# mantasu/face-crop-plus

Hardware: AMD Instinct MI355X
Metric: faces/sec end-to-end (detect+align+crop) (higher is better)
Workload: dtype f16x3; 1 GPU; RetinaFace detect + 5-pt align/crop, batch=32/GPU synthetic 1024x1024 RGB, strategy=largest, det_threshold=0.6, output 256x256, detector on 2 HIP streams x 16 images; global_batch=32, image_size=1024, parallelism=dp1

## Files before the change

face-crop-plus_amd/_native.py:

```python
from __future__ import annotations

import ctypes as C
import os

_HERE = os.path.dirname(os.path.abspath(__file__))
LIB_PATH = os.path.join(_HERE, "csrc", "libfcp_hip.so")
ABI_VERSION = 15

c_f32p = C.c_void_p
_lib = None


class ConvDesc(C.Structure):
    _fields_ = [
        ("in_", C.c_void_p), ("w", C.c_void_p), ("bias", C.c_void_p), ("out", C.c_void_p),
        ("res1", C.c_void_p), ("res2", C.c_void_p), ("wscale", C.c_void_p), ("in2", C.c_void_p),
        ("n", C.c_int32), ("in_h", C.c_int32), ("in_w", C.c_int32),
        ("cin", C.c_int32), ("in_ld", C.c_int32), ("in_up2", C.c_int32),
        ("cout", C.c_int32), ("kh", C.c_int32), ("kw", C.c_int32),
        ("stride", C.c_int32), ("pad", C.c_int32),
        ("out_h", C.c_int32), ("out_w", C.c_int32), ("out_ld", C.c_int32),
        ("tile_n", C.c_int32), ("cin4", C.c_int32),
        ("act_slope", C.c_float), ("alpha", C.c_float), ("alpha2", C.c_float),
        ("res1_pre", C.c_int32), ("res1_ld", C.c_int32), ("res1_h", C.c_int32),
        ("res1_w", C.c_int32), ("res2_ld", C.c_int32), ("precision", C.c_int32),
        ("in_fmt", C.c_int32), ("out_fmt", C.c_int32), ("res1_fmt", C.c_int32), ("res2_fmt", C.c_int32),
        ("tile_m", C.c_int32), ("cin2", C.c_int32), ("in2_ld", C.c_int32), ("in2_h", C.c_int32),
        ("in2_w", C.c_int32), ("in2_stride", C.c_int32), ("flags", C.c_int32), ("cu_budget", C.c_int32),
        ("band_top", C.c_int32), ("band_bottom", C.c_int32),
    ]


CONV_FLAT_ADDR = 1
CONV_BALANCE_TAIL = 2
CHAIN_OUT_EVEN_ONLY = 1


class ChainDesc(C.Structure):
    _fields_ = [(k, C.c_void_p) for k in ("t1", "w2", "ws2", "b2", "w3", "ws3", "b3", "res", "out", "w1n", "ws1n",
                                          "b1n", "t1n", "t1b")] + \
               [(k, C.c_int32) for k in ("n", "h", "w", "c", "cn", "t1_ld", "res_ld", "out_ld", "t1n_ld", "nout", "tile_m", "flags",
                                         "cb", "t1b_ld", "t1b_h", "t1b_w", "t1b_stride")]


_P, _I, _F, _L = C.c_void_p, C.c_int, C.c_float, C.c_int64
SIGNATURES = {
    "fcp_conv2d_nhwc_f32": [C.POINTER(ConvDesc), _P],
    "fcp_bottleneck_chain_f16x3": [C.POINTER(ChainDesc), _P],
    "fcp_u8_to_nhwc4_f32": [_P, _P, _L, C.POINTER(C.c_float), _F, _P],
    "fcp_f32nchw_to_nhwc4_f32": [_P, _P, _I, _I, _I, C.POINTER(C.c_float), _F, _P],
    "fcp_maxpool3x3s2_nhwc_f32": [_P, _P, _I, _I, _I, _I, _I, _I, _I, _P],
    "fcp_maxpool3x3s2_split32": [_P, _P, _I, _I, _I, _I, _I, _I, _I, _P],
    "fcp_stem7x7s2_relu_pool_u8": [_P, _I, _I, _I, C.POINTER(C.c_int32), _P, _P, _P, _P, _I, _I, _P],
    "fcp_stem7x7s2_relu_pool_conv1_u8": [_P, _I, _I, _I, C.POINTER(C.c_int32), _P, _P, _P, _P, _I, _I, _P, _P, _P, _P, _I, _P],
    "fcp_stem7x7s2_relu_pool_f32": [_P, _I, _I, _I, _P, _P, _P, _P, _I, _I, _P],
    "fcp_f32_to_split32": [_P, _P, _L, _I, _P],
    "fcp_split32_to_f32": [_P, _P, _L, _I, _P],
    "fcp_absmax_nhwc": [_P, _L, _I, _I, _I, _P, _P],
    "fcp_retina_decode": [_P, _P, _P, _I, _I, _I, _F, _F, _F, _P, _P, _P, _P, _P, _P, _P, _P, _P],
    "fcp_retina_nms_select": [_P, _P, _P, _I, _I, _F, _I, _P, _P, _P, _P, _P, _P],
    "fcp_retina_gather_faces": [_P, _P, _P, _I, _I, _P, _I, _P, _P, _P, _P],
    "fcp_estimate_transform": [_P, _P, _I, _I, _I, _P, _P, _P],
    "fcp_estimate_transform_counted": [_P, _P, _I, _I, _I, _P, _P, _P, _P, _P],
    "fcp_bise_preprocess_u8": [_P, _I, _I, _I, _P, _I, _I, C.POINTER(C.c_float), C.POINTER(C.c_float), _P],
    "fcp_avgpool_nhwc_f32": [_P, _I, _I, _I, _I, _P, _P],
    "fcp_fc_f32": [_P, _P, _P, _P, _I, _I, _I, _I, _P, _P],
    "fcp_scale_add_nhwc_f32": [_P, _I, _P, _P, _P, _I, _I, _I, _I, _P, _I, _P],
    "fcp_parse_tail": [_P, _I, _I, _I, _I, _I, _I, _I, _I, _I, _P, _P, _P],
    "fcp_label_mask_u8": [_P, _L, C.c_uint32, _P, _P],
    "fcp_bicubic_down4_u8": [_P, _I, _I, _I, _P, _P],
    "fcp_warp_affine_u8": [_P, _I, _I, _I, _P, _P, _P, _P, _I, _I, _I, _I, _P, _P],
    "fcp_warp_affine_u8_float": [_P, _I, _I, _I, _P, _P, _P, _P, _I, _I, _I, _I, _P, _P],
    "fcp_build_batch_u8": [_P, _L, _P, _P, _I, _I, _I, _I, _P, _P],
    "fcp_warp_affine_u8_ragged": [_P, _L, _P, _P, _P, _P, _I, _I, _I, _I, _P, _P],
    "fcp_warp_affine_u8_float_ragged": [_P, _L, _P, _P, _P, _P, _I, _I, _I, _I, _P, _P],
    "fcp_resize_area_ragged_u8": [_P, _L, _P, _P, _I, _P, _L, _P],
    "fcp_warp_affine_u8_interp": [_P, _I, _I, _I, _P, _P, _P, _P, _I, _I, _I, _I, _I, _P, _P],
    "fcp_warp_affine_u8_interp_ragged": [_P, _L, _P, _P, _P, _P, _I, _I, _I, _I, _I, _P, _P],
    "fcp_warp_interp_weights": [_I, _P],
    "fcp_crop_sharpness_u8": [_P, _I, _I, _I, _P, _P, _P],
    "fcp_jpeg_encode_u8": [_P, _I, _I, _I, _I, _I, _I, _P, _L, _L, _P, _P, _L, _P],
    "fcp_jpeg_encode_ex_u8": [_P, _I, _I, _I, _I, _I, _I, _I, _P, _L, _L, _P, _P, _P, _L, _P],
    "fcp_jpeg_huffman_tables": [_P, _I, _P, _P, _P],
    "fcp_png_encode_u8": [_P, _I, _I, _I, _I, _P, _L, _L, _P, _P, _L, _P],
    "fcp_png_huffman_lengths": [_P, _I, _P, _P, _P],
    "fcp_matte_u8": [_P, _P, _I, _I, _I, C.c_uint32, _I, _I, _I, _I, _P, _P, _P],
    "fcp_clahe_u8": [_P, _I, _I, _I, _I, C.c_double, _P, _P, _P],
    "fcp_matte_blur_u8": [_P, _P, _I, _I, _I, C.c_uint32, _I, _P, _I, _P, _P, _P, _L, _P],
    "fcp_matte_refine_u8": [_P, _P, _I, _I, _I, C.c_uint32, _I, _I, _P, _P, _L, _P],
    "fcp_matte_alpha_u8": [_P, _P, _I, _I, _I, _I, _I, _I, _P, _P],
    "fcp_matte_blur_alpha_u8": [_P, _P, _P, _I, _I, _I, C.c_uint32, _P, _I, _P, _P, _L, _P],
    "fcp_subject_mask_u8": [_P, _I, _I, _I, C.c_uint32, _I, _I, _P, _P, _L, _P],
    "fcp_feather_alpha_u8": [_P, _I, _I, _I, C.c_uint32, _I, _P, _P],
    "fcp_cutout_u8": [_P, _P, _I, _I, _I, _I, _I, _I, _I, _P, _I, _P, _P, _L, _P],
}
EXPORTS = ["fcp_abi_version", "fcp_last_error", "fcp_retina_nms_workspace_bytes", "fcp_jpeg_workspace_bytes",
           "fcp_jpeg_workspace_bytes_ex", "fcp_matte_blur_workspace_bytes", "fcp_matte_refine_workspace_bytes",
           "fcp_subject_mask_workspace_bytes", "fcp_png_workspace_bytes", "fcp_cutout_workspace_bytes"] + list(SIGNATURES)


def lib():
    global _lib
    if _lib is not None:
        return _lib
    if not os.path.isfile(LIB_PATH):
        raise RuntimeError(
            f"HIP extension not built: {LIB_PATH} is missing. Run "
            f"`python face-crop-plus_amd/build_native.py` (needs hipcc). There is no CPU fallback.")
    l = C.CDLL(LIB_PATH)
    l.fcp_abi_version.restype = C.c_int
    l.fcp_last_error.restype = C.c_char_p
    if l.fcp_abi_version() != ABI_VERSION:
        raise RuntimeError(f"libfcp_hip.so ABI {l.fcp_abi_version()} != expected {ABI_VERSION}; rebuild")
    l.fcp_retina_nms_workspace_bytes.argtypes = [C.c_int, C.c_int]
    l.fcp_retina_nms_workspace_bytes.restype = C.c_int64
    l.fcp_jpeg_workspace_bytes.argtypes = [C.c_int, C.c_int, C.c_int, C.c_int]
    l.fcp_jpeg_workspace_bytes.restype = C.c_int64
    l.fcp_jpeg_workspace_bytes_ex.argtypes = [C.c_int] * 6
    l.fcp_jpeg_workspace_bytes_ex.restype = C.c_int64
    l.fcp_png_workspace_bytes.argtypes = [C.c_int, C.c_int, C.c_int, C.c_int]
    l.fcp_png_workspace_bytes.restype = C.c_int64
    l.fcp_matte_blur_workspace_bytes.argtypes = [C.c_int, C.c_int, C.c_int]
    l.fcp_matte_blur_workspace_bytes.restype = C.c_int64
    l.fcp_matte_refine_workspace_bytes.argtypes = [C.c_int, C.c_int, C.c_int]
    l.fcp_matte_refine_workspace_bytes.restype = C.c_int64
    l.fcp_subject_mask_workspace_bytes.argtypes = [C.c_int, C.c_int, C.c_int]
    l.fcp_subject_mask_workspace_bytes.restype = C.c_int64
    l.fcp_cutout_workspace_bytes.argtypes = [C.c_int, C.c_int, C.c_int]
    l.fcp_cutout_workspace_bytes.restype = C.c_int64
    for name, args in SIGNATURES.items():
        fn = getattr(l, name)
        fn.argtypes = args
        fn.restype = C.c_int
    _lib = l
    return l


def check(rc: int, what: str = ""):
    if rc != 0:
        msg = lib().fcp_last_error().decode(errors="replace")
        raise RuntimeError(f"{what or 'fcp_hip'} failed ({rc}): {msg}")


def stream_ptr():
    import torch
    return C.c_void_p(torch.cuda.current_stream().cuda_stream)


def ptr(t, byte_offset: int = 0):
    if t is None:
        return C.c_void_p(0)
    return C.c_void_p(t.data_ptr() + byte_offset)
```

face-crop-plus_amd/csrc/fcp_retina_post.hip:

```cpp
#include "fcp_common.h"
#include "fcp_hip.h"

namespace {

constexpr int DEC_THREADS = 1024;
constexpr int NMS_THREADS = 1024;
constexpr int SORT_LDS_KEYS = 8192;
constexpr int NMS_ALIVE_WORDS = SORT_LDS_KEYS - 256;
constexpr int NMS_LDS_CAP = NMS_ALIVE_WORDS * 64;
constexpr int NMS_MAX_CAP = 1 << 26;

struct Levels {
  int h[3], w[3], start[4];
};

__device__ __forceinline__ int ceil_div(int a, int b) { return (a + b - 1) / b; }

constexpr int DEC_MAX_ROUNDS = 64;

struct Decoded {
  float score, box[4], ldm[10];
};

__device__ __forceinline__ const float* head_cell(const float* head0, const float* head1, const float* head2, const Levels& lv,
                                                  int img, int p, int& l, int& cell, int& a) {
  l = p >= lv.start[2] ? 2 : (p >= lv.start[1] ? 1 : 0);
  const int q = p - lv.start[l];
  cell = q >> 1; a = q & 1;
  return (l == 0 ? head0 : (l == 1 ? head1 : head2)) + ((long)img * lv.h[l] * lv.w[l] + cell) * 32;
}

__device__ __forceinline__ float face_score(const float* hp, int a) {
  const float l0 = hp[2 * a], l1 = hp[2 * a + 1];
  const float mx = fmaxf(l0, l1);
  const float e0 = expf(l0 - mx), e1 = expf(l1 - mx);
  const float inv = 1.0f / (e0 + e1);
  return e1 * inv;
}

__device__ __forceinline__ void decode_prior(const float* hp, const Levels& lv, int l, int cell, int a, int img_h, int img_w,
                                             float v0, float v1, Decoded& d) {
  const float fw = (float)img_w, fh = (float)img_h;
  const int wl = lv.w[l];
  const int i = cell / wl, j = cell - i * wl;
  const int step = 8 << l;
  const double ms = (double)((16 << (2 * l)) << a);
  const float pcx = (float)(((double)j + 0.5) * (double)step / (double)img_w);
  const float pcy = (float)(((double)i + 0.5) * (double)step / (double)img_h);
  const float pw = (float)(ms / (double)img_w);
  const float ph = (float)(ms / (double)img_h);
  d.score = face_score(hp, a);
  const float* bp = hp + 4 + 4 * a;
  const float cx = pcx + (bp[0] * v0) * pw;
  const float cy = pcy + (bp[1] * v0) * ph;
  const float bw = pw * expf(bp[2] * v1);
  const float bh = ph * expf(bp[3] * v1);
  const float x1 = cx - bw / 2.0f, y1 = cy - bh / 2.0f;
  const float x2 = bw + x1, y2 = bh + y1;
  d.box[0] = x1 * fw; d.box[1] = y1 * fh; d.box[2] = x2 * fw; d.box[3] = y2 * fh;
  const float* lp = hp + 12 + 10 * a;
#pragma unroll
  for (int k = 0; k < 5; ++k) {
    d.ldm[2 * k] = (pcx + (lp[2 * k] * v0) * pw) * fw;
    d.ldm[2 * k + 1] = (pcy + (lp[2 * k + 1] * v0) * ph) * fh;
  }
}

__global__ void __launch_bounds__(DEC_THREADS) retina_decode_kernel(
    const float* __restrict__ head0, const float* __restrict__ head1, const float* __restrict__ head2,
    Levels lv, int img_h, int img_w, float thr, float v0, float v1, float* __restrict__ cand_score,
    float* __restrict__ cand_box, float* __restrict__ cand_ldm, int* __restrict__ cand_prior,
    int* __restrict__ cand_count, float* __restrict__ dense_score, float* __restrict__ dense_box,
    float* __restrict__ dense_ldm) {
  constexpr int NWAVE = DEC_THREADS / 64;
  __shared__ int cnt[DEC_MAX_ROUNDS * NWAVE];
  const int img = blockIdx.x;
  const int tid = threadIdx.x, lane = tid & 63, wave = tid >> 6;
  const int P = lv.start[3];
  const int rounds_all = (P + DEC_THREADS - 1) / DEC_THREADS;
  __shared__ int s_total;
  int total = 0;

  for (int r0 = 0; r0 < rounds_all; r0 += DEC_MAX_ROUNDS) {
    const int rounds = min(DEC_MAX_ROUNDS, rounds_all - r0);
    unsigned long long passbits = 0ull;
    for (int r = 0; r < rounds; ++r) {
      const int p = (r0 + r) * DEC_THREADS + tid;
      bool pass = false;
      if (p < P) {
        int l, cell, a;
        const float* hp = head_cell(head0, head1, head2, lv, img, p, l, cell, a);
        pass = face_score(hp, a) > thr;
      }
      passbits |= pass ? (1ull << r) : 0ull;
      const unsigned long long bal = __ballot(pass);
      if (lane == 0) cnt[r * NWAVE + wave] = __popcll(bal);
    }
    __syncthreads();
    if (wave == 0) {
      int carry = total;
      const int n = rounds * NWAVE;
      for (int base = 0; base < n; base += 64) {
        const int idx = base + lane;
        const int v = idx < n ? cnt[idx] : 0;
        int incl = v;
#pragma unroll
        for (int o = 1; o < 64; o <<= 1) {
          const int t = __shfl_up(incl, o);
          if (lane >= o) incl += t;
        }
        if (idx < n) cnt[idx] = carry + incl - v;
        carry += __shfl(incl, 63);
      }
      if (lane == 0) s_total = carry;
    }
    __syncthreads();
    total = s_total;
    for (int r = 0; r < rounds; ++r) {
      const int p = (r0 + r) * DEC_THREADS + tid;
      const bool pass = (passbits >> r) & 1ull;
      const unsigned long long bal = __ballot(pass);
      if (p >= P || (!pass && dense_score == nullptr)) continue;
      int l, cell, a;
      const float* hp = head_cell(head0, head1, head2, lv, img, p, l, cell, a);
      Decoded dc;
      decode_prior(hp, lv, l, cell, a, img_h, img_w, v0, v1, dc);
      if (dense_score != nullptr) {
        const long d = (long)img * P + p;
        dense_score[d] = dc.score;
#pragma unroll
        for (int k = 0; k < 4; ++k) dense_box[d * 4 + k] = dc.box[k];
#pragma unroll
        for (int k = 0; k < 10; ++k) dense_ldm[d * 10 + k] = dc.ldm[k];
      }
      if (pass) {
        const long d = (long)img * P + cnt[r * NWAVE + wave] + __popcll(bal & ((1ull << lane) - 1ull));
        cand_score[d] = dc.score;
        cand_prior[d] = p;
#pragma unroll
        for (int k = 0; k < 4; ++k) cand_box[d * 4 + k] = dc.box[k];
#pragma unroll
        for (int k = 0; k < 10; ++k) cand_ldm[d * 10 + k] = dc.ldm[k];
      }
    }
    __syncthreads();
  }
  if (tid == 0) cand_count[img] = total;
}

__device__ __forceinline__ void bitonic_pairs(unsigned long long* a, int npairs, int j, int k, int tid,
                                              int nthreads, int index_base) {
  for (int idx = tid; idx < npairs; idx += nthreads) {
    const int i = 2 * j * (idx / j) + (idx % j);
    const int l = i + j;
    const bool asc = (((i + index_base) & k) == 0);
    const unsigned long long x = a[i], y = a[l];
    if ((x > y) == asc) { a[i] = y; a[l] = x; }
  }
}

__device__ __forceinline__ bool suppressed(float kx1, float ky1, float kx2, float ky2, float karea,
                                           float x1, float y1, float x2, float y2, float area, float thr) {
  const float xx1 = fmaxf(kx1, x1), yy1 = fmaxf(ky1, y1);
  const float xx2 = fminf(kx2, x2), yy2 = fminf(ky2, y2);
  const float w = fmaxf(0.0f, xx2 - xx1 + 1.0f);
  const float h = fmaxf(0.0f, yy2 - yy1 + 1.0f);
  const float a = w * h;
  const float ovr = a / (karea + area - a);
  return !(ovr <= thr);
}

template <bool kGlobalAlive>
__device__ __forceinline__ void greedy_nms(unsigned long long* alive, unsigned long long* lkeys, const float* sbox,
                                           const unsigned long long* gkeys, int* kpos, int K, float thr, int& s_kc,
                                           int tid, int lane, int wave) {
  float* tile = reinterpret_cast<float*>(lkeys + NMS_ALIVE_WORDS);
  int* tile_n = reinterpret_cast<int*>(tile + 64 * 5);
  const int nwords = (K + 63) >> 6;
  for (int wd = tid; wd < nwords; wd += NMS_THREADS) {
    const int lo = wd << 6;
    unsigned long long m = 0ull;
    if (lo + 64 <= K) m = ~0ull;
    else if (lo < K) m = (1ull << (K - lo)) - 1ull;
    alive[wd] = m;
  }
  if (tid == 0) s_kc = 0;
  if (kGlobalAlive) __threadfence_block();
  __syncthreads();

  const int ntiles = (K + 63) >> 6;
  for (int t = 0; t < ntiles; ++t) {
    if (wave == 0) {
      const int c = (t << 6) + lane;
      float x1 = 0.f, y1 = 0.f, x2 = 0.f, y2 = 0.f, area = 0.f;
      if (c < K) { x1 = sbox[c * 5]; y1 = sbox[c * 5 + 1]; x2 = sbox[c * 5 + 2]; y2 = sbox[c * 5 + 3]; area = sbox[c * 5 + 4]; }
      bool me = (alive[t] >> lane) & 1ull;
      for (int b = 0; b < 64; ++b) {
        const unsigned long long m = __ballot(me);
        if (!((m >> b) & 1ull)) continue;
        const float kx1 = __shfl(x1, b), ky1 = __shfl(y1, b), kx2 = __shfl(x2, b), ky2 = __shfl(y2, b);
        const float ka = __shfl(area, b);
        if (lane > b && me && suppressed(kx1, ky1, kx2, ky2, ka, x1, y1, x2, y2, area, thr)) me = false;
      }
      const unsigned long long m = __ballot(me);
      const int rank = __popcll(m & ((1ull << lane) - 1ull));
      const int kc = s_kc;
      if (me) {
        kpos[kc + rank] = (int)(unsigned)(gkeys[c] & 0xffffffffull);
        tile[rank * 5 + 0] = x1; tile[rank * 5 + 1] = y1; tile[rank * 5 + 2] = x2; tile[rank * 5 + 3] = y2;
        tile[rank * 5 + 4] = area;
      }
      if (lane == 0) { *tile_n = __popcll(m); s_kc = kc + __popcll(m); }
    }
    __syncthreads();
    const int nk = *tile_n;
    if (nk > 0) {
      for (int wd = t + 1 + wave; wd < nwords && (wd << 6) < K; wd += NMS_THREADS / 64) {
        const unsigned long long m = alive[wd];
        if (m == 0ull) continue;
        bool me = (m >> lane) & 1ull;
        if (me) {
          const int c = (wd << 6) + lane;
          const float x1 = sbox[c * 5], y1 = sbox[c * 5 + 1], x2 = sbox[c * 5 + 2], y2 = sbox[c * 5 + 3];
          const float area = sbox[c * 5 + 4];
          for (int q = 0; q < nk; ++q) {
            if (suppressed(tile[q * 5], tile[q * 5 + 1], tile[q * 5 + 2], tile[q * 5 + 3], tile[q * 5 + 4], x1,
                           y1, x2, y2, area, thr)) { me = false; break; }
          }
        }
        const unsigned long long nm = __ballot(me);
        if (lane == 0) alive[wd] = nm;
      }
    }
    if (kGlobalAlive) __threadfence_block();
    __syncthreads();
  }
}

__global__ void __launch_bounds__(NMS_THREADS) retina_nms_kernel(
    const float* __restrict__ cand_score, const float* __restrict__ cand_box,
    const int* __restrict__ cand_count, int cap, int cap_p2, float thr, int strategy,
    unsigned long long* __restrict__ ws_keys, float* __restrict__ ws_box, unsigned long long* __restrict__ ws_alive,
    int alive_stride, int* __restrict__ keep_pos,
    int* __restrict__ keep_count, int* __restrict__ sel_pos, int* __restrict__ sel_count) {
  __shared__ unsigned long long lkeys[SORT_LDS_KEYS];
  __shared__ int s_kc;
  __shared__ float s_best_area[NMS_THREADS / 64];
  __shared__ int s_best_rank[NMS_THREADS / 64];
  const int img = blockIdx.x, tid = threadIdx.x, lane = tid & 63, wave = tid >> 6;
  const int K = min(cand_count[img], cap);
  const float* score = cand_score + (long)img * cap;
  const float4* box = reinterpret_cast<const float4*>(cand_box) + (long)img * cap;
  int* kpos = keep_pos + (long)img * cap;
  int* spos = sel_pos + (long)img * cap;
  if (K <= 0) {
    if (tid == 0) { keep_count[img] = 0; sel_count[img] = 0; }
    return;
  }
  int Kp = 64;
  while (Kp < K) Kp <<= 1;
  const int nwords = (K + 63) >> 6;
  unsigned long long* gkeys = ws_keys + (long)img * cap_p2;
  float* sbox = ws_box + (long)img * cap_p2 * 5;

  const bool in_lds = Kp <= SORT_LDS_KEYS;
  unsigned long long* keys = in_lds ? lkeys : gkeys;
  for (int i = tid; i < Kp; i += NMS_THREADS) {
    unsigned long long kv = ~0ull;
    if (i < K) kv = ((unsigned long long)(~__float_as_uint(score[i])) << 32) | (unsigned)i;
    keys[i] = kv;
  }
  __syncthreads();
  if (in_lds) {
    for (int k = 2; k <= Kp; k <<= 1)
      for (int j = k >> 1; j > 0; j >>= 1) {
        bitonic_pairs(keys, Kp >> 1, j, k, tid, NMS_THREADS, 0);
        __syncthreads();
      }
  } else {
    for (int k = 2; k <= Kp; k <<= 1) {
      int j = k >> 1;
      for (; j >= SORT_LDS_KEYS; j >>= 1) {
        bitonic_pairs(gkeys, Kp >> 1, j, k, tid, NMS_THREADS, 0);
        __threadfence_block();
        __syncthreads();
      }
      for (int c0 = 0; c0 < Kp; c0 += SORT_LDS_KEYS) {
        for (int i = tid; i < SORT_LDS_KEYS; i += NMS_THREADS) lkeys[i] = gkeys[c0 + i];
        __syncthreads();
        for (int jj = j; jj > 0; jj >>= 1) {
          bitonic_pairs(lkeys, SORT_LDS_KEYS >> 1, jj, k, tid, NMS_THREADS, c0);
          __syncthreads();
        }
        for (int i = tid; i < SORT_LDS_KEYS; i += NMS_THREADS) gkeys[c0 + i] = lkeys[i];
        __syncthreads();
      }
    }
  }
  for (int i = tid; i < K; i += NMS_THREADS) {
    const unsigned long long kv = keys[i];
    const int pos = (int)(unsigned)(kv & 0xffffffffull);
    const float4 b = box[pos];
    const float area = (b.z - b.x + 1.0f) * (b.w - b.y + 1.0f);
    sbox[i * 5 + 0] = b.x; sbox[i * 5 + 1] = b.y; sbox[i * 5 + 2] = b.z; sbox[i * 5 + 3] = b.w;
    sbox[i * 5 + 4] = area;
    if (in_lds) gkeys[i] = kv;
  }
  __threadfence_block();
  __syncthreads();

  if (nwords <= NMS_ALIVE_WORDS)
    greedy_nms<false>(lkeys, lkeys, sbox, gkeys, kpos, K, thr, s_kc, tid, lane, wave);
  else
    greedy_nms<true>(ws_alive + (long)img * alive_stride, lkeys, sbox, gkeys, kpos, K, thr, s_kc, tid, lane, wave);
  const int kc = s_kc;
  if (tid == 0) keep_count[img] = kc;

  if (strategy == 0) {
    for (int i = tid; i < kc; i += NMS_THREADS) spos[i] = kpos[i];
    if (tid == 0) sel_count[img] = kc;
  } else if (strategy == 1) {
    if (tid == 0) { spos[0] = kpos[0]; sel_count[img] = kc > 0 ? 1 : 0; }
  } else {
    float best = -INFINITY; int brank = 0x7fffffff; bool bnan = false;
    __threadfence_block();
    for (int i = tid; i < kc; i += NMS_THREADS) {
      const float4 b = box[kpos[i]];
      const float area = (b.z - b.x + 1.0f) * (b.w - b.y + 1.0f);
      const bool isn = area != area;
      if (bnan) continue;
      if (isn) { bnan = true; best = area; brank = i; }
      else if (brank == 0x7fffffff || area > best) { best = area; brank = i; }
    }
    for (int off = 32; off > 0; off >>= 1) {
      const float oa = __shfl_down(best, off); const int orank = __shfl_down(brank, off);
      const int on = __shfl_down((int)bnan, off);
      bool take;
      if (orank == 0x7fffffff) take = false;
      else if (brank == 0x7fffffff) take = true;
      else if (on != (int)bnan) take = on != 0;
      else if (bnan) take = orank < brank;
      else take = (oa > best) || (oa == best && orank < brank);
      if (take) { best = oa; brank = orank; bnan = on != 0; }
    }
    if (lane == 0) { s_best_area[wave] = best; s_best_rank[wave] = bnan ? -brank - 1 : brank; }
    __syncthreads();
    if (tid == 0) {
      float fb = 0.f; int fr = 0x7fffffff; bool fn = false;
      for (int wv = 0; wv < NMS_THREADS / 64; ++wv) {
        int rk = s_best_rank[wv]; const float ar = s_best_area[wv];
        if (rk == 0x7fffffff) continue;
        const bool isn = rk < 0;
        if (isn) rk = -rk - 1;
        bool take;
        if (fr == 0x7fffffff) take = true;
        else if (isn != fn) take = isn;
        else if (isn) take = rk < fr;
        else take = (ar > fb) || (ar == fb && rk < fr);
        if (take) { fb = ar; fr = rk; fn = isn; }
      }
      if (kc > 0) { spos[0] = kpos[fr]; sel_count[img] = 1; } else sel_count[img] = 0;
    }
  }
}

__global__ void __launch_bounds__(64) retina_gather_kernel(
    const float* __restrict__ cand_ldm, const int* __restrict__ sel_pos, const int* __restrict__ sel_count,
    int n, int cap, const int* __restrict__ paddings, int max_faces, int* __restrict__ face_offset,
    float* __restrict__ out_ldm, int* __restrict__ out_img) {
  const int img = blockIdx.x, lane = threadIdx.x;
  int before = 0, all = 0;
  for (int i = lane; i < n; i += 64) {
    const int c = sel_count[i];
    all += c;
    before += i < img ? c : 0;
  }
#pragma unroll
  for (int o = 32; o > 0; o >>= 1) {
    before += __shfl_xor(before, o);
    all += __shfl_xor(all, o);
  }
  const int off = before, cnt = sel_count[img];
  if (lane == 0) {
    face_offset[img] = off;
    if (img == n - 1) face_offset[n] = all;
  }
  const float px = paddings ? (float)paddings[img * 4 + 2] : 0.f;
  const float py = paddings ? (float)paddings[img * 4 + 0] : 0.f;
  for (int e = lane; e < cnt * 10; e += 64) {
    const int k = e / 10, c = e - k * 10;
    const int face = off + k;
    if (face >= max_faces) break;
    const float v = cand_ldm[((long)img * cap + sel_pos[(long)img * cap + k]) * 10 + c];
    out_ldm[(long)face * 10 + c] = v - ((c & 1) ? py : px);
    if (c == 0) out_img[face] = img;
  }
  for (long face = (long)all + img; face < max_faces; face += n) {
    if (lane < 10) out_ldm[face * 10 + lane] = 0.f;
    if (lane == 10) out_img[face] = 0;
  }
}

inline int pow2_ceil(int v) { int p = 64; while (p < v) p <<= 1; return p; }

}

extern "C" int64_t fcp_retina_nms_workspace_bytes(int n, int cap) {
  if (n <= 0 || cap <= 0 || cap > NMS_MAX_CAP) return 0;
  const int64_t cap_p2 = pow2_ceil(cap);
  return (int64_t)n * cap_p2 * (8 + 5 * 4) + (cap > NMS_LDS_CAP ? (int64_t)n * (cap_p2 / 64) * 8 : 0);
}

extern "C" int fcp_retina_decode(const float* head0, const float* head1, const float* head2, int n,
                                 int img_h, int img_w, float vis_threshold, float var0, float var1,
                                 float* cand_score, float* cand_box, float* cand_ldm, int32_t* cand_prior,
                                 int32_t* cand_count, float* dense_score, float* dense_box,
                                 float* dense_ldm, fcp_stream_t stream) {
  FCP_REQUIRE(head0 && head1 && head2, "retina_decode: null head pointer");
  FCP_REQUIRE(cand_score && cand_box && cand_ldm && cand_prior && cand_count, "retina_decode: null output");
  FCP_REQUIRE(n > 0 && img_h > 0 && img_w > 0, "retina_decode: bad sizes");
  FCP_REQUIRE((dense_score == nullptr) == (dense_box == nullptr) && (dense_box == nullptr) == (dense_ldm == nullptr),
              "retina_decode: dense outputs must be all set or all NULL");
  Levels lv;
  lv.start[0] = 0;
  for (int l = 0; l < 3; ++l) {
    const int s = 8 << l;
    lv.h[l] = (img_h + s - 1) / s;
    lv.w[l] = (img_w + s - 1) / s;
    lv.start[l + 1] = lv.start[l] + 2 * lv.h[l] * lv.w[l];
  }
  hipLaunchKernelGGL(retina_decode_kernel, dim3(n), dim3(DEC_THREADS), 0, (hipStream_t)stream, head0, head1,
                     head2, lv, img_h, img_w, vis_threshold, var0, var1, cand_score, cand_box, cand_ldm,
                     cand_prior, cand_count, dense_score, dense_box, dense_ldm);
  FCP_LAUNCH_OK();
  return 0;
}

extern "C" int fcp_retina_nms_select(const float* cand_score, const float* cand_box,
                                     const int32_t* cand_count, int n, int cap, float nms_threshold,
                                     int strategy, void* workspace, int32_t* keep_pos, int32_t* keep_count,
                                     int32_t* sel_pos, int32_t* sel_count, fcp_stream_t stream) {
  FCP_REQUIRE(cand_score && cand_box && cand_count && workspace, "retina_nms: null input");
  FCP_REQUIRE(keep_pos && keep_count && sel_pos && sel_count, "retina_nms: null output");
  FCP_REQUIRE(n > 0 && cap > 0, "retina_nms: bad sizes");
  FCP_REQUIRE(cap <= NMS_MAX_CAP, "retina_nms: capacity above %d candidates per image is not supported", NMS_MAX_CAP);
  FCP_REQUIRE(strategy >= 0 && strategy <= 2, "Unsupported startegy: %d", strategy);
  FCP_REQUIRE(((uintptr_t)cand_box & 15) == 0 && ((uintptr_t)workspace & 7) == 0, "retina_nms: misaligned buffers");
  const int cap_p2 = pow2_ceil(cap);
  unsigned long long* keys = reinterpret_cast<unsigned long long*>(workspace);
  float* sbox = reinterpret_cast<float*>(keys + (size_t)n * cap_p2);
  unsigned long long* alive = cap > NMS_LDS_CAP ? reinterpret_cast<unsigned long long*>(sbox + (size_t)n * cap_p2 * 5) : nullptr;
  hipLaunchKernelGGL(retina_nms_kernel, dim3(n), dim3(NMS_THREADS), 0, (hipStream_t)stream, cand_score,
                     cand_box, cand_count, cap, cap_p2, nms_threshold, strategy, keys, sbox, alive, cap_p2 / 64, keep_pos,
                     keep_count, sel_pos, sel_count);
  FCP_LAUNCH_OK();
  return 0;
}

extern "C" int fcp_retina_gather_faces(const float* cand_ldm, const int32_t* sel_pos,
                                       const int32_t* sel_count, int n, int cap, const int32_t* paddings,
                                       int max_faces, int32_t* face_offset, float* out_ldm,
                                       int32_t* out_img, fcp_stream_t stream) {
  FCP_REQUIRE(cand_ldm && sel_pos && sel_count && face_offset && out_ldm && out_img, "retina_gather: null pointer");
  FCP_REQUIRE(n > 0 && cap > 0 && max_faces > 0, "retina_gather: bad sizes");
  hipLaunchKernelGGL(retina_gather_kernel, dim3(n), dim3(64), 0, (hipStream_t)stream, cand_ldm, sel_pos,
                     sel_count, n, cap, paddings, max_faces, face_offset, out_ldm, out_img);
  FCP_LAUNCH_OK();
  return 0;
}
```

face-crop-plus_amd/csrc/torch_ops/fcp_torch_ops.cpp:

```cpp
#include <ATen/ATen.h>
#include <ATen/hip/HIPContext.h>
#include <c10/core/DeviceGuard.h>
#include <torch/library.h>

#include <climits>
#include <tuple>

#include "fcp_hip.h"

namespace {

using at::Tensor;

void* cur_stream() { return (void*)at::hip::getCurrentHIPStream().stream(); }

#define FCP_DEVICE_GUARD(t) const c10::OptionalDeviceGuard fcp_guard_(at::device_of(t))

void ok(int rc, const char* what) { TORCH_CHECK(rc == 0, what, " failed (", rc, "): ", fcp_last_error()); }

const Tensor& dev(const Tensor& t, const char* name, at::ScalarType dt) {
  TORCH_CHECK(t.is_cuda(), name, " must live on the GPU");
  TORCH_CHECK(t.scalar_type() == dt, name, " has dtype ", t.scalar_type(), ", expected ", dt);
  TORCH_CHECK(t.is_contiguous(), name, " must be contiguous");
  return t;
}
template <typename T>
const T* optp(const c10::optional<Tensor>& t, const char* name, at::ScalarType dt) {
  if (!t.has_value() || !t->defined()) return nullptr;
  return dev(*t, name, dt).data_ptr<T>();
}

Tensor conv2d_impl(const Tensor& x, int64_t x_c0, int64_t cin, const Tensor& w, const c10::optional<Tensor>& bias,
                   const c10::optional<Tensor>& wscale, const c10::optional<Tensor>& res1, int64_t res1_c0,
                   const c10::optional<Tensor>& res2, int64_t res2_c0, const c10::optional<Tensor>& out_, int64_t out_c0,
                   int64_t cout, int64_t kh, int64_t kw, int64_t stride, int64_t pad, double act_slope, double alpha,
                   double alpha2, bool res1_pre, int64_t precision, int64_t in_fmt, int64_t out_fmt, int64_t res1_fmt,
                   int64_t res2_fmt, bool in_up2, bool cin4, int64_t tile_m, int64_t tile_n, const c10::optional<Tensor>& x2,
                   int64_t x2_c0, int64_t cin2, int64_t x2_stride, int64_t flags, int64_t cu_budget, int64_t band_top,
                   int64_t band_bottom) {
  dev(x, "x", at::kFloat);
  FCP_DEVICE_GUARD(x);
  TORCH_CHECK(x.dim() == 4, "x must be NHWC (n, h, w, ld)");
  TORCH_CHECK(w.is_cuda() && w.is_contiguous(), "w must be a contiguous GPU tensor (packed filter)");
  const int64_t n = x.size(0), ph = x.size(1), pw = x.size(2), ld = x.size(3);
  const int64_t ih = in_up2 ? 2 * ph : ph, iw = in_up2 ? 2 * pw : pw;
  const int64_t oh = (ih - band_top - band_bottom + 2 * pad - kh) / stride + 1, ow = (iw + 2 * pad - kw) / stride + 1;
  Tensor out = out_.has_value() && out_->defined() ? *out_ : at::empty({n, oh, ow, cout}, x.options());
  dev(out, "out", at::kFloat);
  TORCH_CHECK(out.dim() == 4 && out.size(0) == n && out.size(1) == oh && out.size(2) == ow && out_c0 + cout <= out.size(3),
              "out has the wrong geometry");
  TORCH_CHECK(x_c0 + (cin4 ? 4 : cin - cin2) <= ld, "input channel view exceeds the buffer");
  fcp_conv_desc d = {};
  d.in = x.data_ptr<float>() + x_c0;
  d.w = w.data_ptr();
  d.bias = optp<float>(bias, "bias", at::kFloat);
  d.wscale = optp<float>(wscale, "wscale", at::kFloat);
  d.out = out.data_ptr<float>() + out_c0;
  d.n = (int)n; d.in_h = (int)ih; d.in_w = (int)iw; d.cin = (int)cin; d.in_ld = (int)ld; d.in_up2 = in_up2;
  d.cout = (int)cout; d.kh = (int)kh; d.kw = (int)kw; d.stride = (int)stride; d.pad = (int)pad;
  d.out_h = (int)oh; d.out_w = (int)ow; d.out_ld = (int)out.size(3);
  d.tile_n = (int)tile_n; d.tile_m = (int)tile_m; d.cin4 = cin4;
  d.act_slope = (float)act_slope; d.alpha = (float)alpha; d.alpha2 = (float)alpha2;
  d.res1_pre = res1_pre; d.precision = (int)precision;
  d.in_fmt = (int)in_fmt; d.out_fmt = (int)out_fmt; d.res1_fmt = (int)res1_fmt; d.res2_fmt = (int)res2_fmt;
  if (res1.has_value() && res1->defined()) {
    dev(*res1, "res1", at::kFloat);
    d.res1 = res1->data_ptr<float>() + res1_c0;
    d.res1_ld = (int)res1->size(3); d.res1_h = (int)res1->size(1); d.res1_w = (int)res1->size(2);
  }
  if (res2.has_value() && res2->defined()) {
    dev(*res2, "res2", at::kFloat);
    d.res2 = res2->data_ptr<float>() + res2_c0;
    d.res2_ld = (int)res2->size(3);
  }
  if (x2.has_value() && x2->defined()) {
    dev(*x2, "x2", at::kFloat);
    d.in2 = x2->data_ptr<float>() + x2_c0;
    d.cin2 = (int)cin2; d.in2_ld = (int)x2->size(3); d.in2_h = (int)x2->size(1); d.in2_w = (int)x2->size(2);
    d.in2_stride = (int)x2_stride;
  }
  d.flags = (int)flags;
  d.cu_budget = (int)cu_budget;
  d.band_top = (int)band_top; d.band_bottom = (int)band_bottom;
  ok(fcp_conv2d_nhwc_f32(&d, cur_stream()), "fcp::conv2d");
  return out;
}

Tensor conv2d(const Tensor& x, int64_t x_c0, int64_t cin, const Tensor& w, const c10::optional<Tensor>& bias,
              const c10::optional<Tensor>& wscale, const c10::optional<Tensor>& res1, int64_t res1_c0,
              const c10::optional<Tensor>& res2, int64_t res2_c0, int64_t cout, int64_t kh, int64_t kw, int64_t stride,
              int64_t pad, double act_slope, double alpha, double alpha2, bool res1_pre, int64_t precision, int64_t in_fmt,
              int64_t out_fmt, int64_t res1_fmt, int64_t res2_fmt, bool in_up2, bool cin4, int64_t tile_m, int64_t tile_n,
              const c10::optional<Tensor>& x2, int64_t x2_c0, int64_t cin2, int64_t x2_stride, int64_t flags, int64_t cu_budget,
              int64_t band_top, int64_t band_bottom) {
  return conv2d_impl(x, x_c0, cin, w, bias, wscale, res1, res1_c0, res2, res2_c0, c10::nullopt, 0, cout, kh, kw, stride, pad,
                     act_slope, alpha, alpha2, res1_pre, precision, in_fmt, out_fmt, res1_fmt, res2_fmt, in_up2, cin4, tile_m,
                     tile_n, x2, x2_c0, cin2, x2_stride, flags, cu_budget, band_top, band_bottom);
}

void conv2d_out(const Tensor& x, int64_t x_c0, int64_t cin, const Tensor& w, const c10::optional<Tensor>& bias,
                const c10::optional<Tensor>& wscale, const c10::optional<Tensor>& res1, int64_t res1_c0,
                const c10::optional<Tensor>& res2, int64_t res2_c0, Tensor& out, int64_t out_c0, int64_t cout, int64_t kh,
                int64_t kw, int64_t stride, int64_t pad, double act_slope, double alpha, double alpha2, bool res1_pre,
                int64_t precision, int64_t in_fmt, int64_t out_fmt, int64_t res1_fmt, int64_t res2_fmt, bool in_up2, bool cin4,
                int64_t tile_m, int64_t tile_n, const c10::optional<Tensor>& x2, int64_t x2_c0, int64_t cin2,
                int64_t x2_stride, int64_t flags, int64_t cu_budget, int64_t band_top, int64_t band_bottom) {
  conv2d_impl(x, x_c0, cin, w, bias, wscale, res1, res1_c0, res2, res2_c0, out, out_c0, cout, kh, kw, stride, pad, act_slope,
              alpha, alpha2, res1_pre, precision, in_fmt, out_fmt, res1_fmt, res2_fmt, in_up2, cin4, tile_m, tile_n, x2, x2_c0,
              cin2, x2_stride, flags, cu_budget, band_top, band_bottom);
}

std::tuple<Tensor, Tensor> bottleneck_chain(const Tensor& t1, int64_t t1_c0, const c10::optional<Tensor>& res, int64_t res_c0,
                                            const c10::optional<Tensor>& w2, const c10::optional<Tensor>& ws2,
                                            const c10::optional<Tensor>& b2, const Tensor& w3, const Tensor& ws3,
                                            const Tensor& b3, const c10::optional<Tensor>& w1n,
                                            const c10::optional<Tensor>& ws1n, const c10::optional<Tensor>& b1n, int64_t c, int64_t nout, int64_t cn, int64_t tile_m, int64_t flags,
                                            const c10::optional<Tensor>& t1b, int64_t t1b_c0, int64_t cb, int64_t t1b_stride) {
  dev(t1, "t1", at::kFloat);
  FCP_DEVICE_GUARD(t1);
  const bool two = t1b.has_value() && t1b->defined();
  TORCH_CHECK(t1.dim() == 4 && t1_c0 + c - (two ? cb : 0) <= t1.size(3), "t1 (n,h,w,>=c) split32 buffer");
  const bool has_res = res.has_value() && res->defined();
  if (has_res) {
    dev(*res, "res", at::kFloat);
    TORCH_CHECK(res->dim() == 4 && res_c0 + nout <= res->size(3), "res (n,h,w,>=nout) split32 buffer");
  }
  Tensor out = at::empty({t1.size(0), t1.size(1), t1.size(2), nout}, t1.options());
  Tensor t1n = at::empty({t1.size(0), t1.size(1), t1.size(2), cn}, t1.options());
  fcp_chain_desc d = {};
  d.t1 = t1.data_ptr<float>() + t1_c0; d.out = out.data_ptr<float>(); d.t1n = t1n.data_ptr<float>();
  if (has_res) { d.res = res->data_ptr<float>() + res_c0; d.res_ld = (int)res->size(3); }
  if (w2.has_value() && w2->defined()) {
    d.w2 = w2->data_ptr(); d.ws2 = optp<float>(ws2, "ws2", at::kFloat); d.b2 = optp<float>(b2, "b2", at::kFloat);
  }
  d.w3 = w3.data_ptr(); d.ws3 = dev(ws3, "ws3", at::kFloat).data_ptr<float>(); d.b3 = dev(b3, "b3", at::kFloat).data_ptr<float>();
  const bool has_next = w1n.has_value() && w1n->defined();
  TORCH_CHECK(has_next == (cn > 0), "w1n / ws1n / b1n are given exactly when cn > 0 (cn == 0: the expand form)");
  if (has_next) {
    d.w1n = w1n->data_ptr(); d.ws1n = optp<float>(ws1n, "ws1n", at::kFloat); d.b1n = optp<float>(b1n, "b1n", at::kFloat);
    TORCH_CHECK(d.ws1n && d.b1n, "ws1n and b1n accompany w1n");
  } else {
    d.t1n = nullptr;
  }
  d.n = (int)t1.size(0); d.h = (int)t1.size(1); d.w = (int)t1.size(2); d.c = (int)c; d.cn = (int)cn; d.nout = (int)nout;
  d.t1_ld = (int)t1.size(3); d.out_ld = (int)nout; d.t1n_ld = (int)cn; d.tile_m = (int)tile_m; d.flags = (int)flags;
  if (two) {
    dev(*t1b, "t1b", at::kFloat);
    TORCH_CHECK(t1b->dim() == 4 && t1b->size(0) == t1.size(0) && t1b_c0 + cb <= t1b->size(3), "t1b (n,hb,wb,>=cb) split32 buffer");
    d.t1b = t1b->data_ptr<float>() + t1b_c0; d.cb = (int)cb; d.t1b_ld = (int)t1b->size(3);
    d.t1b_h = (int)t1b->size(1); d.t1b_w = (int)t1b->size(2); d.t1b_stride = (int)t1b_stride;
  }
  ok(fcp_bottleneck_chain_f16x3(&d, cur_stream()), "fcp::bottleneck_chain");
  return {out, t1n};
}

std::tuple<Tensor, Tensor, Tensor, Tensor, Tensor> retina_decode(const Tensor& h0, const Tensor& h1, const Tensor& h2,
                                                                 int64_t img_h, int64_t img_w, double vis, double var0,
                                                                 double var1) {
  dev(h0, "head0", at::kFloat); dev(h1, "head1", at::kFloat); dev(h2, "head2", at::kFloat);
  FCP_DEVICE_GUARD(h0);
  TORCH_CHECK(img_h > 0 && img_w > 0, "image size must be positive");
  TORCH_CHECK(h0.dim() == 4, "head maps are (n, ceil(h/s), ceil(w/s), 32) fp32 NHWC");
  const int64_t n = h0.size(0);
  int64_t P = 0;
  const Tensor* heads[3] = {&h0, &h1, &h2};
  int li = 0;
  for (int64_t s : {8, 16, 32}) {
    const Tensor& h = *heads[li++];
    const int64_t fh = (img_h + s - 1) / s, fw = (img_w + s - 1) / s;
    TORCH_CHECK(h.dim() == 4 && h.size(0) == n && h.size(1) == fh && h.size(2) == fw && h.size(3) == 32,
                "head map of stride ", s, " must be (", n, ", ", fh, ", ", fw, ", 32) for a ", img_h, " x ", img_w, " image, got ",
                h.sizes());
    P += 2 * fh * fw;
  }
  auto f = h0.options();
  auto i = h0.options().dtype(at::kInt);
  Tensor score = at::empty({n, P}, f), box = at::empty({n, P, 4}, f), ldm = at::empty({n, P, 10}, f);
  Tensor prior = at::empty({n, P}, i), count = at::empty({n}, i);
  ok(fcp_retina_decode(h0.data_ptr<float>(), h1.data_ptr<float>(), h2.data_ptr<float>(), (int)n, (int)img_h, (int)img_w,
                       (float)vis, (float)var0, (float)var1, score.data_ptr<float>(), box.data_ptr<float>(),
                       ldm.data_ptr<float>(), prior.data_ptr<int>(), count.data_ptr<int>(), nullptr, nullptr, nullptr,
                       cur_stream()), "fcp::retina_decode");
  return {score, box, ldm, prior, count};
}

std::tuple<Tensor, Tensor, Tensor, Tensor> nms_select(const Tensor& score, const Tensor& box, const Tensor& count,
                                                      double thr, int64_t strategy) {
  dev(score, "cand_score", at::kFloat); dev(box, "cand_box", at::kFloat); dev(count, "cand_count", at::kInt);
  FCP_DEVICE_GUARD(score);
  TORCH_CHECK(score.dim() == 2, "cand_score is (n, cap)");
  const int64_t n = score.size(0), cap = score.size(1);
  TORCH_CHECK(box.dim() == 3 && box.size(0) == n && box.size(1) == cap && box.size(2) == 4, "cand_box must be (", n, ", ", cap,
              ", 4), got ", box.sizes());
  TORCH_CHECK(count.dim() == 1 && count.size(0) == n, "cand_count must be (", n, ",), got ", count.sizes());
  TORCH_CHECK(strategy >= 0 && strategy <= 2, "strategy: 0 all, 1 best, 2 largest");
  auto i = score.options().dtype(at::kInt);
  Tensor ws = at::empty({fcp_retina_nms_workspace_bytes((int)n, (int)cap)}, score.options().dtype(at::kByte));
  Tensor keep_pos = at::empty({n, cap}, i), keep_count = at::empty({n}, i), sel_pos = at::empty({n, cap}, i), sel_count = at::empty({n}, i);
  ok(fcp_retina_nms_select(score.data_ptr<float>(), box.data_ptr<float>(), count.data_ptr<int>(), (int)n, (int)cap, (float)thr,
                           (int)strategy, ws.data_ptr(), keep_pos.data_ptr<int>(), keep_count.data_ptr<int>(),
                           sel_pos.data_ptr<int>(), sel_count.data_ptr<int>(), cur_stream()), "fcp::nms_select");
  return {keep_pos, keep_count, sel_pos, sel_count};
}

std::tuple<Tensor, Tensor, Tensor> gather_faces(const Tensor& ldm, const Tensor& sel_pos, const Tensor& sel_count,
                                                const c10::optional<Tensor>& paddings, int64_t max_faces) {
  dev(ldm, "cand_ldm", at::kFloat); dev(sel_pos, "sel_pos", at::kInt); dev(sel_count, "sel_count", at::kInt);
  FCP_DEVICE_GUARD(ldm);
  TORCH_CHECK(sel_pos.dim() == 2, "sel_pos is (n, cap)");
  const int64_t n = sel_pos.size(0), cap = sel_pos.size(1);
  TORCH_CHECK(ldm.dim() == 3 && ldm.size(0) == n && ldm.size(1) == cap && ldm.size(2) == 10, "cand_ldm must be (", n, ", ", cap,
              ", 10), got ", ldm.sizes());
  TORCH_CHECK(sel_count.dim() == 1 && sel_count.size(0) == n, "sel_count must be (", n, ",), got ", sel_count.sizes());
  TORCH_CHECK(max_faces >= 1, "max_faces must be >= 1");
  if (paddings.has_value() && paddings->defined())
    TORCH_CHECK(paddings->dim() == 2 && paddings->size(0) == n && paddings->size(1) == 4, "paddings must be (", n, ", 4)");
  auto i = ldm.options().dtype(at::kInt);
  Tensor off = at::empty({n + 1}, i), out_ldm = at::empty({max_faces, 5, 2}, ldm.options()), out_img = at::empty({max_faces}, i);
  ok(fcp_retina_gather_faces(ldm.data_ptr<float>(), sel_pos.data_ptr<int>(), sel_count.data_ptr<int>(), (int)n, (int)cap,
                             optp<int>(paddings, "paddings", at::kInt), (int)max_faces, off.data_ptr<int>(),
                             out_ldm.data_ptr<float>(), out_img.data_ptr<int>(), cur_stream()), "fcp::gather_faces");
  return {out_ldm, out_img, off};
}

std::tuple<Tensor, Tensor> similarity_from_5pt(const Tensor& src, const Tensor& dst, bool allow_skew,
                                               const c10::optional<Tensor>& face_count,
                                               const c10::optional<Tensor>& valid_total) {
  dev(src, "src", at::kFloat); dev(dst, "dst", at::kFloat);
  FCP_DEVICE_GUARD(src);
  TORCH_CHECK(src.dim() == 3 && src.size(2) == 2 && dst.dim() == 2 && dst.size(0) == src.size(1), "src (f,k,2), dst (k,2)");
  const int64_t f = src.size(0);
  Tensor mat = at::empty({f, 2, 3}, src.options().dtype(at::kDouble)), okf = at::empty({f}, src.options().dtype(at::kInt));
  const int* fc = optp<int>(face_count, "face_count", at::kInt);
  int64_t* vt = const_cast<int64_t*>(optp<int64_t>(valid_total, "valid_total", at::kLong));
  TORCH_CHECK(fc == nullptr || face_count->numel() == 1, "face_count is a scalar");
  TORCH_CHECK(vt == nullptr || valid_total->numel() == 1, "valid_total is a scalar");
  ok(fcp_estimate_transform_counted(src.data_ptr<float>(), dst.data_ptr<float>(), (int)f, (int)src.size(1), allow_skew, fc,
                                    mat.data_ptr<double>(), okf.data_ptr<int>(), vt, cur_stream()),
     "fcp::similarity_from_5pt");
  return {mat, okf};
}


template <class Fn>
Tensor warp_affine_with(Fn fn, const char* what, const Tensor& images, const Tensor& img_idx, const Tensor& mat,
                        const c10::optional<Tensor>& okf, const c10::optional<Tensor>& paddings, int64_t out_w, int64_t out_h,
                        int64_t border) {
  dev(images, "images", at::kByte); dev(img_idx, "img_idx", at::kInt); dev(mat, "mat", at::kDouble);
  FCP_DEVICE_GUARD(images);
  TORCH_CHECK(images.dim() == 4 && images.size(3) == 3, "images (n,h,w,3) uint8");
  const int64_t f = img_idx.size(0);
  TORCH_CHECK(mat.dim() == 3 && mat.size(0) == f && mat.size(1) == 2 && mat.size(2) == 3, "mat must be (", f, ", 2, 3) float64");
  Tensor out = at::empty({f, out_h, out_w, 3}, images.options());
  ok(fn(images.data_ptr<uint8_t>(), (int)images.size(0), (int)images.size(1), (int)images.size(2), img_idx.data_ptr<int>(),
        mat.data_ptr<double>(), optp<int>(okf, "ok", at::kInt), optp<int>(paddings, "paddings", at::kInt), (int)f, (int)out_h,
        (int)out_w, (int)border, out.data_ptr<uint8_t>(), cur_stream()), what);
  return out;
}

Tensor warp_affine_u8(const Tensor& images, const Tensor& img_idx, const Tensor& mat, const c10::optional<Tensor>& okf,
                      const c10::optional<Tensor>& paddings, int64_t out_w, int64_t out_h, int64_t border) {
  return warp_affine_with(fcp_warp_affine_u8, "fcp::warp_affine_u8", images, img_idx, mat, okf, paddings, out_w, out_h, border);
}

Tensor warp_affine_u8_float(const Tensor& images, const Tensor& img_idx, const Tensor& mat, const c10::optional<Tensor>& okf,
                            const c10::optional<Tensor>& paddings, int64_t out_w, int64_t out_h, int64_t border) {
  return warp_affine_with(fcp_warp_affine_u8_float, "fcp::warp_affine_u8_float", images, img_idx, mat, okf, paddings, out_w,
                          out_h, border);
}

Tensor warp_affine_u8_interp(const Tensor& images, const Tensor& img_idx, const Tensor& mat, const c10::optional<Tensor>& okf,
                             const c10::optional<Tensor>& paddings, int64_t out_w, int64_t out_h, int64_t border,
                             int64_t interp) {
  const int ip = (int)interp;
  return warp_affine_with(
      [ip](const uint8_t* im, int n, int h, int w, const int32_t* idx, const double* m, const int32_t* okp, const int32_t* pad,
           int f, int oh, int ow, int b, uint8_t* out, fcp_stream_t st) {
        return fcp_warp_affine_u8_interp(im, n, h, w, idx, m, okp, pad, f, oh, ow, b, ip, out, st);
      },
      "fcp::warp_affine_u8_interp", images, img_idx, mat, okf, paddings, out_w, out_h, border);
}

const Tensor& host_table(const Tensor& t, const char* name, int64_t words) {
  TORCH_CHECK(!t.is_cuda() && t.scalar_type() == at::kLong && t.is_contiguous() && t.dim() == 2 && t.size(1) == words, name,
              " must be a contiguous CPU int64 (n, ", words, ") tensor of records");
  return t;
}

template <class Check, class Fn>
Tensor warp_affine_ragged_with(Check check, Fn fn, const char* what, const Tensor& blob, const Tensor& srcs, const Tensor& mat,
                               const c10::optional<Tensor>& okf, int64_t out_w, int64_t out_h, int64_t border) {
  dev(blob, "blob", at::kByte); dev(mat, "mat", at::kDouble); host_table(srcs, "srcs", 2);
  FCP_DEVICE_GUARD(blob);
  check();
  const int64_t f = srcs.size(0);
  TORCH_CHECK(mat.numel() == f * 6, "mat must hold (", f, ", 6) float64");
  TORCH_CHECK(!okf.has_value() || !okf->defined() || okf->numel() == f, "ok must hold ", f, " flags");
  Tensor srcs_dev = srcs.to(blob.device(), true);
  Tensor out = at::empty({f, out_h, out_w, 3}, blob.options());
  const auto* host = reinterpret_cast<const fcp_warp_src*>(srcs.data_ptr<int64_t>());
  const auto* devp = reinterpret_cast<const fcp_warp_src*>(srcs_dev.data_ptr<int64_t>());
  ok(fn(blob.data_ptr<uint8_t>(), blob.numel(), host, devp, mat.data_ptr<double>(), optp<int>(okf, "ok", at::kInt), (int)f,
        (int)out_h, (int)out_w, (int)border, out.data_ptr<uint8_t>(), cur_stream()),
     what);
  return out;
}

Tensor warp_affine_u8_ragged(const Tensor& blob, const Tensor& srcs, const Tensor& mat, const c10::optional<Tensor>& okf,
                             int64_t out_w, int64_t out_h, int64_t border, int64_t family) {
  return warp_affine_ragged_with(
      [family] { TORCH_CHECK(family == 0 || family == 1, "family must be 0 (fixed) or 1 (float32)"); },
      family == 0 ? fcp_warp_affine_u8_ragged : fcp_warp_affine_u8_float_ragged, "fcp::warp_affine_u8_ragged", blob, srcs,
      mat, okf, out_w, out_h, border);
}

Tensor warp_affine_u8_interp_ragged(const Tensor& blob, const Tensor& srcs, const Tensor& mat, const c10::optional<Tensor>& okf,
                                    int64_t out_w, int64_t out_h, int64_t border, int64_t interp) {
  const int ip = (int)interp;
  return warp_affine_ragged_with(
      [] {},
      [ip](const uint8_t* b, int64_t bytes, const fcp_warp_src* sh, const fcp_warp_src* sd, const double* m, const int32_t* okp,
           int f, int oh, int ow, int bd, uint8_t* out, fcp_stream_t st) {
        return fcp_warp_affine_u8_interp_ragged(b, bytes, sh, sd, m, okp, f, oh, ow, bd, ip, out, st);
      },
      "fcp::warp_affine_u8_interp_ragged", blob, srcs, mat, okf, out_w, out_h, border);
}

void resize_area_u8_ragged(const Tensor& src, const Tensor& levels, const Tensor& dst) {
  dev(src, "src", at::kByte); dev(dst, "dst", at::kByte); host_table(levels, "levels", 4);
  FCP_DEVICE_GUARD(src);
  const int64_t n = levels.size(0);
  if (n == 0) return;
  Tensor levels_dev = levels.to(src.device(), true);
  ok(fcp_resize_area_ragged_u8(src.data_ptr<uint8_t>(), src.numel(),
                               reinterpret_cast<const fcp_area_level*>(levels.data_ptr<int64_t>()),
                               reinterpret_cast<const fcp_area_level*>(levels_dev.data_ptr<int64_t>()), (int)n,
                               dst.data_ptr<uint8_t>(), dst.numel(), cur_stream()),
     "fcp::resize_area_u8_ragged");
}

Tensor crop_sharpness(const Tensor& crops, const c10::optional<Tensor>& okf) {
  dev(crops, "crops", at::kByte);
  FCP_DEVICE_GUARD(crops);
  TORCH_CHECK(crops.dim() == 4 && crops.size(3) == 3, "crops (f,h,w,3) uint8");
  const int64_t f = crops.size(0), h = crops.size(1), w = crops.size(2);
  TORCH_CHECK(f <= INT_MAX && h <= INT_MAX && w <= INT_MAX, "crops (f,h,w,3): sizes past int");
  TORCH_CHECK(!okf.has_value() || !okf->defined() || okf->numel() == f, "ok must hold ", f, " flags");
  Tensor sums = at::empty({f, 2}, crops.options().dtype(at::kLong));
  ok(fcp_crop_sharpness_u8(crops.data_ptr<uint8_t>(), (int)f, (int)h, (int)w, optp<int>(okf, "ok", at::kInt),
                           sums.data_ptr<int64_t>(), cur_stream()),
     "fcp::crop_sharpness");
  return sums;
}

Tensor jpeg_encode(const Tensor& crops, int64_t quality, int64_t subsampling, const Tensor& out) {
  dev(crops, "crops", at::kByte);
  FCP_DEVICE_GUARD(crops);
  TORCH_CHECK((crops.dim() == 4 && (crops.size(3) == 3 || crops.size(3) == 1)) || crops.dim() == 3,
              "crops (f,h,w,3) or (f,h,w) uint8");
  const int64_t f = crops.size(0), h = crops.size(1), w = crops.size(2), c = crops.dim() == 4 ? crops.size(3) : 1;
  TORCH_CHECK(f <= INT_MAX && h <= INT_MAX && w <= INT_MAX, "crops: sizes past int");
  TORCH_CHECK(quality >= INT_MIN && quality <= INT_MAX && subsampling >= INT_MIN && subsampling <= INT_MAX,
              "quality / subsampling past int");
  TORCH_CHECK(out.is_cuda() && out.scalar_type() == at::kByte && out.get_device() == crops.get_device(),
              "out must be a uint8 tensor on the device of the crops");
  TORCH_CHECK(out.dim() == 2 && out.size(0) == f, "out must be (", f, ", capacity)");
  const int64_t capacity = out.size(1), stride = f > 1 ? out.stride(0) : capacity;
  TORCH_CHECK(capacity == 0 || out.stride(1) == 1, "out: the bytes of a row must be contiguous");
  TORCH_CHECK(stride >= capacity, "out: rows overlap");
  Tensor lengths = at::empty({f}, crops.options().dtype(at::kInt));
  const int64_t need = fcp_jpeg_workspace_bytes((int)f, (int)h, (int)w, (int)c);
  ok(need < 0 ? -1 : 0, "fcp::jpeg_encode");
  Tensor work = at::empty({need}, crops.options());
  ok(fcp_jpeg_encode_u8(crops.data_ptr<uint8_t>(), (int)f, (int)h, (int)w, (int)c, (int)quality, (int)subsampling,
                        capacity > 0 ? out.data_ptr<uint8_t>() : nullptr, stride, capacity, lengths.data_ptr<int32_t>(),
                        work.data_ptr(), need, cur_stream()),
     "fcp::jpeg_encode");
  return lengths;
}

Tensor jpeg_encode_ex(const Tensor& crops, int64_t quality, int64_t subsampling, const Tensor& out,
                      const c10::optional<Tensor>& tables) {
  dev(crops, "crops", at::kByte);
  FCP_DEVICE_GUARD(crops);
  TORCH_CHECK((crops.dim() == 4 && (crops.size(3) == 3 || crops.size(3) == 1)) || crops.dim() == 3,
              "crops (f,h,w,3) or (f,h,w) uint8");
  const int64_t f = crops.size(0), h = crops.size(1), w = crops.size(2), c = crops.dim() == 4 ? crops.size(3) : 1;
  TORCH_CHECK(f <= INT_MAX && h <= INT_MAX && w <= INT_MAX, "crops: sizes past int");
  TORCH_CHECK(quality >= INT_MIN && quality <= INT_MAX && subsampling >= INT_MIN && subsampling <= INT_MAX,
              "quality / subsampling past int");
  TORCH_CHECK(out.is_cuda() && out.scalar_type() == at::kByte && out.get_device() == crops.get_device(),
              "out must be a uint8 tensor on the device of the crops");
  TORCH_CHECK(out.dim() == 2 && out.size(0) == f, "out must be (", f, ", capacity)");
  const int64_t capacity = out.size(1), stride = f > 1 ? out.stride(0) : capacity;
  TORCH_CHECK(capacity == 0 || out.stride(1) == 1, "out: the bytes of a row must be contiguous");
  TORCH_CHECK(stride >= capacity, "out: rows overlap");
  const bool optimize = tables.has_value() && tables->defined();
  if (optimize) {
    const Tensor& t = *tables;
    TORCH_CHECK(t.is_cuda() && t.scalar_type() == at::kByte && t.get_device() == crops.get_device() && t.is_contiguous() &&
                    t.dim() == 3 && t.size(0) == f && t.size(1) == 4 && t.size(2) == 272,
                "tables must be a contiguous (", f, ",4,272) uint8 tensor on the device of the crops");
  }
  Tensor lengths = at::empty({f}, crops.options().dtype(at::kInt));
  const int64_t need = fcp_jpeg_workspace_bytes_ex((int)f, (int)h, (int)w, (int)c, (int)subsampling, optimize ? 1 : 0);
  ok(need < 0 ? -1 : 0, "fcp::jpeg_encode_ex");
  Tensor work = at::empty({need}, crops.options());
  ok(fcp_jpeg_encode_ex_u8(crops.data_ptr<uint8_t>(), (int)f, (int)h, (int)w, (int)c, (int)quality, (int)subsampling,
                           optimize ? 1 : 0, capacity > 0 ? out.data_ptr<uint8_t>() : nullptr, stride, capacity,
                           lengths.data_ptr<int32_t>(), optimize ? tables->data_ptr<uint8_t>() : nullptr, work.data_ptr(), need,
                           cur_stream()),
     "fcp::jpeg_encode_ex");
  return lengths;
}

std::tuple<Tensor, Tensor> jpeg_huffman_tables(const Tensor& freq, bool with_codes) {
  dev(freq, "freq", at::kInt);
  FCP_DEVICE_GUARD(freq);
  TORCH_CHECK(freq.dim() == 2 && freq.size(1) == 256 && freq.is_contiguous(), "freq (n,256) int32, contiguous");
  const int64_t n = freq.size(0);
  TORCH_CHECK(n <= INT_MAX, "freq: rows past int");
  Tensor tables = at::empty({n, 272}, freq.options().dtype(at::kByte));
  Tensor codes = with_codes ? at::empty({n, 256}, freq.options()) : at::empty({0}, freq.options());
  ok(fcp_jpeg_huffman_tables(reinterpret_cast<const uint32_t*>(freq.data_ptr<int32_t>()), (int)n, tables.data_ptr<uint8_t>(),
                             with_codes ? reinterpret_cast<uint32_t*>(codes.data_ptr<int32_t>()) : nullptr, cur_stream()),
     "fcp::jpeg_huffman_tables");
  return {tables, codes};
}

Tensor png_encode(const Tensor& pixels, const Tensor& out) {
  dev(pixels, "pixels", at::kByte);
  FCP_DEVICE_GUARD(pixels);
  TORCH_CHECK((pixels.dim() == 4 && (pixels.size(3) == 3 || pixels.size(3) == 4 || pixels.size(3) == 1)) || pixels.dim() == 3,
              "pixels (f,h,w,3), (f,h,w,4) or (f,h,w) uint8");
  const int64_t f = pixels.size(0), h = pixels.size(1), w = pixels.size(2), c = pixels.dim() == 4 ? pixels.size(3) : 1;
  TORCH_CHECK(f <= INT_MAX && h <= INT_MAX && w <= INT_MAX, "pixels: sizes past int");
  TORCH_CHECK(out.is_cuda() && out.scalar_type() == at::kByte && out.get_device() == pixels.get_device(),
              "out must be a uint8 tensor on the device of the pixels");
  TORCH_CHECK(out.dim() == 2 && out.size(0) == f, "out must be (", f, ", capacity)");
  const int64_t capacity = out.size(1), stride = f > 1 ? out.stride(0) : capacity;
  TORCH_CHECK(capacity == 0 || out.stride(1) == 1, "out: the bytes of a row must be contiguous");
  TORCH_CHECK(stride >= capacity, "out: rows overlap");
  Tensor lengths = at::empty({f}, pixels.options().dtype(at::kInt));
  const int64_t need = fcp_png_workspace_bytes((int)f, (int)h, (int)w, (int)c);
  ok(need < 0 ? -1 : 0, "fcp::png_encode");
  Tensor work = at::empty({need}, pixels.options());
  ok(fcp_png_encode_u8(pixels.data_ptr<uint8_t>(), (int)f, (int)h, (int)w, (int)c,
                       capacity > 0 ? out.data_ptr<uint8_t>() : nullptr, stride, capacity, lengths.data_ptr<int32_t>(),
                       work.data_ptr(), need, cur_stream()),
     "fcp::png_encode");
  return lengths;
}

std::tuple<Tensor, Tensor> png_huffman_lengths(const Tensor& freq, bool with_codes) {
  dev(freq, "freq", at::kInt);
  FCP_DEVICE_GUARD(freq);
  TORCH_CHECK(freq.dim() == 2 && freq.size(1) == 286 && freq.is_contiguous(), "freq (n,286) int32, contiguous");
  const int64_t n = freq.size(0);
  TORCH_CHECK(n <= INT_MAX, "freq: rows past int");
  Tensor lengths = at::empty({n, 286}, freq.options().dtype(at::kByte));
  Tensor codes = with_codes ? at::empty({n, 286}, freq.options()) : at::empty({0}, freq.options());
  ok(fcp_png_huffman_lengths(reinterpret_cast<const uint32_t*>(freq.data_ptr<int32_t>()), (int)n, lengths.data_ptr<uint8_t>(),
                             with_codes ? reinterpret_cast<uint32_t*>(codes.data_ptr<int32_t>()) : nullptr, cur_stream()),
     "fcp::png_huffman_lengths");
  return {lengths, codes};
}

static void crops_and_plane(const Tensor& crops, const Tensor& plane, const char* name, int64_t& f, int64_t& h, int64_t& w) {
  TORCH_CHECK(crops.dim() == 4 && crops.size(3) == 3, "crops (f,h,w,3) uint8");
  f = crops.size(0), h = crops.size(1), w = crops.size(2);
  TORCH_CHECK(f <= INT_MAX && h <= INT_MAX && w <= INT_MAX, "crops (f,h,w,3): sizes past int");
  TORCH_CHECK(plane.get_device() == crops.get_device() && plane.dim() == 3 && plane.size(0) == f && plane.size(1) == h &&
                  plane.size(2) == w, name, " must be (", f, ",", h, ",", w, ") uint8 on the device of the crops");
}

static void labels_plane(const Tensor& labels, int64_t class_bits, int64_t& f, int64_t& h, int64_t& w) {
  TORCH_CHECK(labels.dim() == 3, "labels (f,h,w) uint8");
  f = labels.size(0), h = labels.size(1), w = labels.size(2);
  TORCH_CHECK(f <= INT_MAX && h <= INT_MAX && w <= INT_MAX, "labels (f,h,w): sizes past int");
  TORCH_CHECK(class_bits >= 0 && class_bits <= (int64_t)UINT_MAX, "class_bits past 32 bits");
}

static int taps16(const char* name, at::IntArrayRef taps, bool allow_empty, uint16_t (&t16)[49]) {
  const int64_t radius = (int64_t)taps.size() - 1;
  TORCH_CHECK((allow_empty && taps.empty()) || (radius >= 3 && radius <= 48), name, ": taps must be ", allow_empty ? "empty or " : "",
              "t[0..radius] with radius 3..48 (got ", taps.size(), " taps)");
  for (int64_t k = 0; k <= radius; ++k) {
    TORCH_CHECK(taps[k] >= 0 && taps[k] <= 65535, name, ": tap ", k, " past 16 bits");
    t16[k] = (uint16_t)taps[k];
  }
  return taps.empty() ? 0 : (int)radius;
}

static Tensor workspace(int64_t need, const Tensor& like) { return at::empty({need < 0 ? 0 : need}, like.options()); }

std::tuple<Tensor, Tensor> matte(const Tensor& crops, const Tensor& labels, int64_t class_bits, int64_t feather, int64_t bg_r,
                                 int64_t bg_g, int64_t bg_b, bool with_alpha) {
  dev(crops, "crops", at::kByte);
  dev(labels, "labels", at::kByte);
  FCP_DEVICE_GUARD(crops);
  int64_t f, h, w;
  crops_and_plane(crops, labels, "labels", f, h, w);
  TORCH_CHECK(class_bits >= 0 && class_bits <= (int64_t)UINT_MAX, "class_bits past 32 bits");
  for (int64_t v : {feather, bg_r, bg_g, bg_b}) TORCH_CHECK(v >= INT_MIN && v <= INT_MAX, "feather / fill past int");
  Tensor out = at::empty_like(crops);
  Tensor alpha = with_alpha ? at::empty({f, h, w}, crops.options()) : at::empty({0}, crops.options());
  ok(fcp_matte_u8(crops.data_ptr<uint8_t>(), labels.data_ptr<uint8_t>(), (int)f, (int)h, (int)w, (uint32_t)class_bits,
                  (int)feather, (int)bg_r, (int)bg_g, (int)bg_b, out.data_ptr<uint8_t>(),
                  with_alpha ? alpha.data_ptr<uint8_t>() : nullptr, cur_stream()),
     "fcp::matte");
  return {out, alpha};
}

std::tuple<Tensor, Tensor> matte_blur(const Tensor& crops, const Tensor& labels, int64_t class_bits, int64_t feather,
                                      at::IntArrayRef taps, bool with_alpha) {
  dev(crops, "crops", at::kByte);
  dev(labels, "labels", at::kByte);
  FCP_DEVICE_GUARD(crops);
  int64_t f, h, w;
  crops_and_plane(crops, labels, "labels", f, h, w);
  TORCH_CHECK(class_bits >= 0 && class_bits <= (int64_t)UINT_MAX, "class_bits past 32 bits");
  TORCH_CHECK(feather >= INT_MIN && feather <= INT_MAX, "feather past int");
  uint16_t t16[49];
  const int radius = taps16("matte_blur", taps, false, t16);
  Tensor out = at::empty_like(crops);
  Tensor alpha = with_alpha ? at::empty({f, h, w}, crops.options()) : at::empty({0}, crops.options());
  Tensor work = workspace(fcp_matte_blur_workspace_bytes((int)f, (int)h, (int)w), crops);
  ok(fcp_matte_blur_u8(crops.data_ptr<uint8_t>(), labels.data_ptr<uint8_t>(), (int)f, (int)h, (int)w, (uint32_t)class_bits,
                       (int)feather, t16, radius, out.data_ptr<uint8_t>(), with_alpha ? alpha.data_ptr<uint8_t>() : nullptr,
                       work.data_ptr(), work.numel(), cur_stream()),
     "fcp::matte_blur");
  return {out, alpha};
}

Tensor matte_refine(const Tensor& crops, const Tensor& labels, int64_t class_bits, int64_t radius, int64_t eps) {
  dev(crops, "crops", at::kByte);
  dev(labels, "labels", at::kByte);
  FCP_DEVICE_GUARD(crops);
  int64_t f, h, w;
  crops_and_plane(crops, labels, "labels", f, h, w);
  TORCH_CHECK(class_bits >= 0 && class_bits <= (int64_t)UINT_MAX, "class_bits past 32 bits");
  for (int64_t v : {radius, eps}) TORCH_CHECK(v >= INT_MIN && v <= INT_MAX, "radius / eps past int");
  Tensor alpha = at::empty({f, h, w}, crops.options());
  Tensor work = workspace(fcp_matte_refine_workspace_bytes((int)f, (int)h, (int)w), crops);
  ok(fcp_matte_refine_u8(crops.data_ptr<uint8_t>(), labels.data_ptr<uint8_t>(), (int)f, (int)h, (int)w, (uint32_t)class_bits,
                         (int)radius, (int)eps, alpha.data_ptr<uint8_t>(), work.data_ptr(), work.numel(), cur_stream()),
     "fcp::matte_refine");
  return alpha;
}

Tensor matte_alpha(const Tensor& crops, const Tensor& alpha, int64_t bg_r, int64_t bg_g, int64_t bg_b) {
  dev(crops, "crops", at::kByte);
  dev(alpha, "alpha", at::kByte);
  FCP_DEVICE_GUARD(crops);
  int64_t f, h, w;
  crops_and_plane(crops, alpha, "alpha", f, h, w);
  for (int64_t v : {bg_r, bg_g, bg_b}) TORCH_CHECK(v >= INT_MIN && v <= INT_MAX, "fill past int");
  Tensor out = at::empty_like(crops);
  ok(fcp_matte_alpha_u8(crops.data_ptr<uint8_t>(), alpha.data_ptr<uint8_t>(), (int)f, (int)h, (int)w, (int)bg_r, (int)bg_g,
                        (int)bg_b, out.data_ptr<uint8_t>(), cur_stream()),
     "fcp::matte_alpha");
  return out;
}

Tensor matte_blur_alpha(const Tensor& crops, const Tensor& labels, const Tensor& alpha, int64_t class_bits, at::IntArrayRef taps) {
  dev(crops, "crops", at::kByte);
  dev(labels, "labels", at::kByte);
  dev(alpha, "alpha", at::kByte);
  FCP_DEVICE_GUARD(crops);
  int64_t f, h, w;
  crops_and_plane(crops, labels, "labels", f, h, w);
  crops_and_plane(crops, alpha, "alpha", f, h, w);
  TORCH_CHECK(class_bits >= 0 && class_bits <= (int64_t)UINT_MAX, "class_bits past 32 bits");
  uint16_t t16[49];
  const int radius = taps16("matte_blur_alpha", taps, false, t16);
  Tensor out = at::empty_like(crops);
  Tensor work = workspace(fcp_matte_blur_workspace_bytes((int)f, (int)h, (int)w), crops);
  ok(fcp_matte_blur_alpha_u8(crops.data_ptr<uint8_t>(), labels.data_ptr<uint8_t>(), alpha.data_ptr<uint8_t>(), (int)f, (int)h,
                             (int)w, (uint32_t)class_bits, t16, radius, out.data_ptr<uint8_t>(), work.data_ptr(), work.numel(),
                             cur_stream()),
     "fcp::matte_blur_alpha");
  return out;
}

Tensor feather_alpha(const Tensor& labels, int64_t class_bits, int64_t feather) {
  dev(labels, "labels", at::kByte);
  FCP_DEVICE_GUARD(labels);
  int64_t f, h, w;
  labels_plane(labels, class_bits, f, h, w);
  TORCH_CHECK(feather >= INT_MIN && feather <= INT_MAX, "feather past int");
  Tensor alpha = at::empty_like(labels);
  ok(fcp_feather_alpha_u8(labels.data_ptr<uint8_t>(), (int)f, (int)h, (int)w, (uint32_t)class_bits, (int)feather,
                          alpha.data_ptr<uint8_t>(), cur_stream()),
     "fcp::feather_alpha");
  return alpha;
}

Tensor cutout(const Tensor& crops, const Tensor& alpha, int64_t mode, int64_t bg_r, int64_t bg_g, int64_t bg_b, at::IntArrayRef taps) {
  dev(crops, "crops", at::kByte);
  dev(alpha, "alpha", at::kByte);
  FCP_DEVICE_GUARD(crops);
  int64_t f, h, w;
  crops_and_plane(crops, alpha, "alpha", f, h, w);
  for (int64_t v : {mode, bg_r, bg_g, bg_b}) TORCH_CHECK(v >= INT_MIN && v <= INT_MAX, "mode / fill past int");
  uint16_t t16[49] = {};
  const int radius = taps16("cutout", taps, true, t16);
  Tensor out = at::empty({f, h, w, mode == FCP_CUTOUT_RGBA ? 4 : 3}, crops.options());
  Tensor work = workspace(taps.empty() ? 0 : fcp_cutout_workspace_bytes((int)f, (int)h, (int)w), crops);
  ok(fcp_cutout_u8(crops.data_ptr<uint8_t>(), alpha.data_ptr<uint8_t>(), (int)f, (int)h, (int)w, (int)mode, (int)bg_r, (int)bg_g,
                   (int)bg_b, t16, radius, out.data_ptr<uint8_t>(), work.data_ptr(), work.numel(), cur_stream()),
     "fcp::cutout");
  return out;
}

Tensor subject_mask(const Tensor& labels, int64_t class_bits, bool keep_largest, int64_t max_hole) {
  dev(labels, "labels", at::kByte);
  FCP_DEVICE_GUARD(labels);
  int64_t f, h, w;
  labels_plane(labels, class_bits, f, h, w);
  TORCH_CHECK(max_hole >= INT_MIN && max_hole <= INT_MAX, "max_hole past int");
  Tensor out = at::empty_like(labels);
  Tensor work = workspace(fcp_subject_mask_workspace_bytes((int)f, (int)h, (int)w), labels);
  ok(fcp_subject_mask_u8(labels.data_ptr<uint8_t>(), (int)f, (int)h, (int)w, (uint32_t)class_bits, keep_largest ? 1 : 0,
                         (int)max_hole, out.data_ptr<uint8_t>(), work.data_ptr(), work.numel(), cur_stream()),
     "fcp::subject_mask");
  return out;
}

Tensor clahe(const Tensor& crops, int64_t grid, double clip_limit) {
  dev(crops, "crops", at::kByte);
  FCP_DEVICE_GUARD(crops);
  TORCH_CHECK(crops.dim() == 4 && crops.size(3) == 3, "crops (f,h,w,3) uint8");
  const int64_t f = crops.size(0), h = crops.size(1), w = crops.size(2);
  TORCH_CHECK(f <= INT_MAX && h <= INT_MAX && w <= INT_MAX, "crops (f,h,w,3): sizes past int");
  TORCH_CHECK(grid >= 1 && grid <= 16, "clahe: grid must be 1..16 (got ", grid, ")");
  Tensor out = at::empty_like(crops);
  Tensor luts = at::empty({f, grid, grid, 256}, crops.options());
  ok(fcp_clahe_u8(crops.data_ptr<uint8_t>(), (int)f, (int)h, (int)w, (int)grid, clip_limit, luts.data_ptr<uint8_t>(),
                  out.data_ptr<uint8_t>(), cur_stream()),
     "fcp::clahe");
  return out;
}

Tensor bicubic_down4_round(const Tensor& x4) {
  dev(x4, "x4", at::kFloat);
  FCP_DEVICE_GUARD(x4);
  TORCH_CHECK(x4.dim() == 3 && x4.size(0) % 4 == 0 && x4.size(1) % 4 == 0 && x4.size(2) >= 3, "x4 (4h,4w,ld>=3) fp32");
  const int64_t h = x4.size(0) / 4, w = x4.size(1) / 4;
  Tensor out = at::empty({h, w, 3}, x4.options().dtype(at::kByte));
  ok(fcp_bicubic_down4_u8(x4.data_ptr<float>(), (int)h, (int)w, (int)x4.size(2), out.data_ptr<uint8_t>(), cur_stream()),
     "fcp::bicubic_down4_round");
  return out;
}

std::tuple<Tensor, Tensor> parse_argmax_hist(const Tensor& logits, int64_t ncls, int64_t mid_h, int64_t mid_w, int64_t out_h,
                                             int64_t out_w) {
  dev(logits, "logits", at::kFloat);
  FCP_DEVICE_GUARD(logits);
  TORCH_CHECK(logits.dim() == 4 && logits.size(3) >= ncls, "logits (f,lh,lw,ld>=ncls)");
  const int64_t f = logits.size(0);
  Tensor labels = at::empty({f, out_h, out_w}, logits.options().dtype(at::kByte));
  Tensor counts = at::empty({f, ncls}, logits.options().dtype(at::kInt));
  ok(fcp_parse_tail(logits.data_ptr<float>(), (int)f, (int)logits.size(1), (int)logits.size(2), (int)logits.size(3), (int)ncls,
                    (int)mid_h, (int)mid_w, (int)out_h, (int)out_w, labels.data_ptr<uint8_t>(), counts.data_ptr<int>(), cur_stream()),
     "fcp::parse_argmax_hist");
  return {labels, counts};
}

}

TORCH_LIBRARY(fcp, m) {
  m.def("conv2d(Tensor x, int x_c0, int cin, Tensor w, Tensor? bias, Tensor? wscale, Tensor? res1, int res1_c0, Tensor? res2, "
        "int res2_c0, int cout, int kh, int kw, int stride, int pad, float act_slope, float alpha, "
        "float alpha2, bool res1_pre, int precision, int in_fmt, int out_fmt, int res1_fmt, int res2_fmt, bool in_up2, "
        "bool cin4, int tile_m, int tile_n, Tensor? x2, int x2_c0, int cin2, int x2_stride, int flags, int cu_budget=0, int band_top=0, "
        "int band_bottom=0) -> Tensor");
  m.def("conv2d_out(Tensor x, int x_c0, int cin, Tensor w, Tensor? bias, Tensor? wscale, Tensor? res1, int res1_c0, Tensor? res2, "
        "int res2_c0, Tensor(a!) out, int out_c0, int cout, int kh, int kw, int stride, int pad, float act_slope, float alpha, "
        "float alpha2, bool res1_pre, int precision, int in_fmt, int out_fmt, int res1_fmt, int res2_fmt, bool in_up2, "
        "bool cin4, int tile_m, int tile_n, Tensor? x2, int x2_c0, int cin2, int x2_stride, int flags, int cu_budget=0, int band_top=0, "
        "int band_bottom=0) -> ()");
  m.def("bottleneck_chain(Tensor t1, int t1_c0, Tensor? res, int res_c0, Tensor? w2, Tensor? ws2, Tensor? b2, Tensor w3, Tensor ws3, "
        "Tensor b3, Tensor? w1n, Tensor? ws1n, Tensor? b1n, int c, int nout, int cn, int tile_m=0, int flags=0, Tensor? t1b=None, "
        "int t1b_c0=0, int cb=0, int t1b_stride=1) -> (Tensor, Tensor)");
  m.def("retina_decode(Tensor head0, Tensor head1, Tensor head2, int img_h, int img_w, float vis, float var0, float var1) "
        "-> (Tensor, Tensor, Tensor, Tensor, Tensor)");
  m.def("nms_select(Tensor cand_score, Tensor cand_box, Tensor cand_count, float nms_threshold, int strategy) "
        "-> (Tensor, Tensor, Tensor, Tensor)");
  m.def("gather_faces(Tensor cand_ldm, Tensor sel_pos, Tensor sel_count, Tensor? paddings, int max_faces) -> (Tensor, Tensor, Tensor)");
  m.def("similarity_from_5pt(Tensor src, Tensor dst, bool allow_skew, Tensor? face_count=None, Tensor(a!)? valid_total=None) "
        "-> (Tensor, Tensor)");
  m.def("warp_affine_u8(Tensor images, Tensor img_idx, Tensor mat, Tensor? ok, Tensor? paddings, int out_w, int out_h, int border) -> Tensor");
  m.def("warp_affine_u8_float(Tensor images, Tensor img_idx, Tensor mat, Tensor? ok, Tensor? paddings, int out_w, int out_h, "
        "int border) -> Tensor");
  m.def("warp_affine_u8_ragged(Tensor blob, Tensor srcs, Tensor mat, Tensor? ok, int out_w, int out_h, int border, int family) "
        "-> Tensor");
  m.def("warp_affine_u8_interp(Tensor images, Tensor img_idx, Tensor mat, Tensor? ok, Tensor? paddings, int out_w, int out_h, "
        "int border, int interp) -> Tensor");
  m.def("warp_affine_u8_interp_ragged(Tensor blob, Tensor srcs, Tensor mat, Tensor? ok, int out_w, int out_h, int border, "
        "int interp) -> Tensor");
  m.def("resize_area_u8_ragged(Tensor src, Tensor levels, Tensor(a!) dst) -> ()");
  m.def("crop_sharpness(Tensor crops, Tensor? ok) -> Tensor");
  m.def("jpeg_encode(Tensor crops, int quality, int subsampling, Tensor(a!) out) -> Tensor");
  m.def("jpeg_encode_ex(Tensor crops, int quality, int subsampling, Tensor(a!) out, Tensor(b!)? tables) -> Tensor");
  m.def("jpeg_huffman_tables(Tensor freq, bool with_codes) -> (Tensor, Tensor)");
  m.def("png_encode(Tensor pixels, Tensor(a!) out) -> Tensor");
  m.def("png_huffman_lengths(Tensor freq, bool with_codes) -> (Tensor, Tensor)");
  m.def("matte(Tensor crops, Tensor labels, int class_bits, int feather, int bg_r, int bg_g, int bg_b, bool with_alpha) "
        "-> (Tensor, Tensor)");
  m.def("clahe(Tensor crops, int grid, float clip_limit) -> Tensor");
  m.def("matte_blur(Tensor crops, Tensor labels, int class_bits, int feather, int[] taps, bool with_alpha) -> (Tensor, Tensor)");
  m.def("matte_refine(Tensor crops, Tensor labels, int class_bits, int radius, int eps) -> Tensor");
  m.def("matte_alpha(Tensor crops, Tensor alpha, int bg_r, int bg_g, int bg_b) -> Tensor");
  m.def("matte_blur_alpha(Tensor crops, Tensor labels, Tensor alpha, int class_bits, int[] taps) -> Tensor");
  m.def("subject_mask(Tensor labels, int class_bits, bool keep_largest, int max_hole) -> Tensor");
  m.def("feather_alpha(Tensor labels, int class_bits, int feather) -> Tensor");
  m.def("cutout(Tensor crops, Tensor alpha, int mode, int bg_r, int bg_g, int bg_b, int[] taps) -> Tensor");
  m.def("bicubic_down4_round(Tensor x4) -> Tensor");
  m.def("parse_argmax_hist(Tensor logits, int ncls, int mid_h, int mid_w, int out_h, int out_w) -> (Tensor, Tensor)");
  m.def("abi_version() -> (int, int)", []() -> std::tuple<int64_t, int64_t> {
    return {(int64_t)FCP_ABI_VERSION, (int64_t)fcp_abi_version()};
  });
}

TORCH_LIBRARY_IMPL(fcp, CUDA, m) {
  m.impl("conv2d", &conv2d);
  m.impl("conv2d_out", &conv2d_out);
  m.impl("bottleneck_chain", &bottleneck_chain);
  m.impl("retina_decode", &retina_decode);
  m.impl("nms_select", &nms_select);
  m.impl("gather_faces", &gather_faces);
  m.impl("similarity_from_5pt", &similarity_from_5pt);
  m.impl("warp_affine_u8", &warp_affine_u8);
  m.impl("warp_affine_u8_float", &warp_affine_u8_float);
  m.impl("warp_affine_u8_ragged", &warp_affine_u8_ragged);
  m.impl("warp_affine_u8_interp", &warp_affine_u8_interp);
  m.impl("warp_affine_u8_interp_ragged", &warp_affine_u8_interp_ragged);
  m.impl("resize_area_u8_ragged", &resize_area_u8_ragged);
  m.impl("crop_sharpness", &crop_sharpness);
  m.impl("jpeg_encode", &jpeg_encode);
  m.impl("jpeg_encode_ex", &jpeg_encode_ex);
  m.impl("jpeg_huffman_tables", &jpeg_huffman_tables);
  m.impl("png_encode", &png_encode);
  m.impl("png_huffman_lengths", &png_huffman_lengths);
  m.impl("matte", &matte);
  m.impl("clahe", &clahe);
  m.impl("matte_blur", &matte_blur);
  m.impl("matte_refine", &matte_refine);
  m.impl("matte_alpha", &matte_alpha);
  m.impl("matte_blur_alpha", &matte_blur_alpha);
  m.impl("subject_mask", &subject_mask);
  m.impl("feather_alpha", &feather_alpha);
  m.impl("cutout", &cutout);
  m.impl("bicubic_down4_round", &bicubic_down4_round);
  m.impl("parse_argmax_hist", &parse_argmax_hist);
}
```

face-crop-plus_amd/retinaface.py:

```python
from __future__ import annotations


import os
import threading

import numpy as np
import torch

from . import _native as N
from . import engine as E
from . import torch_ops as T
from .weights import load_state_dict

STRATEGIES = {"all": 0, "best": 1, "largest": 2}


class RetinaFace:
    WEIGHTS_FILENAME = "retinaface_detector.pth"

    def __init__(self, strategy: str = "all", vis: float = 0.6):
        self.strategy = strategy
        self.vis_threshold = vis
        self.nms_threshold = 0.4
        self.variance = [0.1, 0.2]
        self.device = None
        self._p = None
        self.precision = 0
        self.fused_chain = True
        self.streams = int(os.environ.get("FCP_DET_STREAMS", "2"))
        self.min_images_per_stream = 6
        self._tls = threading.local()

    def load(self, device: str | torch.device = "cuda:0", weights=None, precision=None):
        device = torch.device(device)
        if device.type != "cuda":
            raise RuntimeError("face_crop_plus_amd runs on an AMD GPU only (device must be cuda:N / hip); "
                               "there is no CPU fallback")
        N.lib()
        self.device = device
        sd = load_state_dict("retinaface", weights, device=device)
        self._repack(sd, precision)
        E.device_props(device)
        E.selfcheck_at_load(self, sd, weights, precision, lambda: self._repack(sd, "f32"))
        return self

    def _repack(self, sd, precision):
        with torch.cuda.device(self.device), E.default_precision(precision):
            self._p = self._pack(sd, self.device)
        self.precision = E.resolve_precision(precision)

    @torch.no_grad()
    def selfcheck(self, sd=None, images_u8: torch.Tensor | None = None, rel_tol: float = 1e-4):
        if self.precision != 1:
            self.selfcheck_report = {"skipped": "exact-fp32 path: nothing to guard"}
            return self.selfcheck_report
        dev = self.device
        with torch.cuda.device(dev):
            if images_u8 is None:
                g = torch.Generator(device="cpu").manual_seed(20260928)
                s = 256
                ramp = (torch.arange(s)[:, None] + torch.arange(s)[None, :]).clamp(max=255).to(torch.uint8)
                images_u8 = torch.stack([torch.randint(0, 256, (s, s, 3), generator=g, dtype=torch.uint8),
                                         torch.full((s, s, 3), 255, dtype=torch.uint8), torch.zeros((s, s, 3), dtype=torch.uint8),
                                         ramp[..., None].expand(s, s, 3).contiguous()]).to(dev)
            images_u8 = images_u8.to(dev).contiguous()
            tuning, E.Autotune.enabled = E.Autotune.enabled, False
            try:
                with E.RangeMonitor() as mon:
                    heads = self.forward_heads(None, images_u8) if "stem_fused" in self._p else \
                        self.forward_heads(E.u8_to_nhwc4(images_u8, sub=(123.0, 117.0, 104.0)))
                rep = {"launch_absmax": mon.check("RetinaFace"), "limit": E.RangeMonitor.LIMIT, "head_rel_diff": None}
                if sd is not None:
                    twin = RetinaFace(self.strategy, self.vis_threshold)
                    twin.device, twin.precision = dev, 0
                    with E.default_precision("f32"):
                        twin._p = self._pack(sd, dev)
                    ref = twin.forward_heads(E.u8_to_nhwc4(images_u8, sub=(123.0, 117.0, 104.0)))
                    rep["head_rel_diff"] = [E.selfcheck_compare("RetinaFace head maps", a.buf, b.buf, rel_tol)
                                            for a, b in zip(heads, ref)]
                    del twin, ref
                    torch.cuda.empty_cache()
            finally:
                E.Autotune.enabled = tuning
        self.selfcheck_report = rep
        return rep

    @staticmethod
    def _pack(sd, dev):
        p = {}
        pc, bn = E.pack_conv, E.bn_of
        p["stem"] = pc(sd["body.conv1.weight"], None, bn(sd, "body.bn1"), 2, 3, dev, cin_perm=[2, 1, 0])
        if E.DEFAULT_PRECISION == 1:
            p["stem_fused"] = E.pack_stem_fused(sd["body.conv1.weight"], bn(sd, "body.bn1"), dev, cin_perm=[2, 1, 0])
        blocks = []
        for li, nb in enumerate((3, 4, 6, 3), 1):
            for b in range(nb):
                pre = f"body.layer{li}.{b}"
                stride = 2 if (b == 0 and li > 1) else 1
                blk = {
                    "c1": pc(sd[pre + ".conv1.weight"], None, bn(sd, pre + ".bn1"), 1, 0, dev),
                    "c2": pc(sd[pre + ".conv2.weight"], None, bn(sd, pre + ".bn2"), stride, 1, dev),
                    "c3": pc(sd[pre + ".conv3.weight"], None, bn(sd, pre + ".bn3"), 1, 0, dev),
                    "ds": None, "feat": (b == nb - 1 and li >= 2),
                }
                if (pre + ".downsample.0.weight") in sd:
                    blk["ds"] = pc(sd[pre + ".downsample.0.weight"], None, bn(sd, pre + ".downsample.1"),
                                   stride, 0, dev)
                    if stride == 1 or E.DEFAULT_PRECISION == 1:
                        fold = lambda cw, cb: E.fold_bn(sd[pre + cw].numpy(), {q: v.numpy() for q, v in bn(sd, pre + cb).items()}, None)
                        (w3, b3), (wd, bd) = fold(".conv3.weight", ".bn3"), fold(".downsample.0.weight", ".downsample.1")
                        blk["c3ds"] = pc(np.concatenate([w3, wd], 1), b3 + bd, None, 1, 0, dev)
                blocks.append(blk)
        p["blocks"] = blocks
        for i in (1, 2, 3):
            p[f"fpn.output{i}"] = pc(sd[f"fpn.output{i}.0.weight"], None, bn(sd, f"fpn.output{i}.1"), 1, 0, dev)
        for i in (1, 2):
            p[f"fpn.merge{i}"] = pc(sd[f"fpn.merge{i}.0.weight"], None, bn(sd, f"fpn.merge{i}.1"), 1, 1, dev)
        head_perm = list(range(0, 128)) + list(range(192, 256)) + list(range(128, 192))
        for k in (1, 2, 3):
            def folded(nm):
                return E.fold_bn(sd[f"ssh{k}.{nm}.0.weight"].numpy(), {q: v.numpy() for q, v in bn(sd, f"ssh{k}.{nm}.1").items()}, None)
            w_b, b_b = folded("conv5X5_1")
            w_a, b_a = folded("conv3X3")
            p[f"ssh{k}.ab"] = pc(np.concatenate([w_b, w_a]), np.concatenate([b_b, b_a]), None, 1, 1, dev)
            w_c, b_c = folded("conv5X5_2")
            w_d, b_d = folded("conv7X7_2")
            p[f"ssh{k}.cd"] = pc(np.concatenate([w_c, w_d]), np.concatenate([b_c, b_d]), None, 1, 1, dev)
            w_e, b_e = folded("conv7x7_3")
            p[f"ssh{k}.e"] = pc(w_e, b_e, None, 1, 1, dev)
            i = k - 1
            hw = np.concatenate([sd[f"{h}.{i}.conv1x1.weight"].numpy() for h in ("ClassHead", "BboxHead", "LandmarkHead")])
            hb = np.concatenate([sd[f"{h}.{i}.conv1x1.bias"].numpy() for h in ("ClassHead", "BboxHead", "LandmarkHead")])
            p[f"head{k}"] = pc(hw, hb, None, 1, 0, dev, cin_perm=head_perm)
        return p

    def forward_heads(self, x4: E.Act | None, images_u8: torch.Tensor | None = None, heads_out=None):
        p = self._p
        f = 1 if self.precision == 1 else 0
        stem_t1 = None
        if images_u8 is not None and "stem_fused" in p:
            n, h, w, _ = images_u8.shape
            hp, wp = ((h - 1) // 2) // 2 + 1, ((w - 1) // 2) // 2 + 1
            cat = E.Act.empty(n, hp, wp, 128, images_u8.device, f)
            c1 = p["blocks"][0]["c1"]
            if f == 1 and E.stem_conv1_supported(c1):
                x, stem_t1 = E.stem_relu_pool_u8(p["stem_fused"], images_u8, cat.slice(64, 64), conv1=c1)
            else:
                x = E.stem_relu_pool_u8(p["stem_fused"], images_u8, cat.slice(64, 64))
        else:
            x = E.conv(p["stem"], x4, act_slope=0.0, out_fmt=f)
            cat = E.Act.empty(x.n, (x.h + 1) // 2, (x.w + 1) // 2, 2 * x.c, x.buf.device, f)
            x = E.maxpool3x3s2(x, cat.slice(x.c, x.c))
        feats = []
        blocks, pre = p["blocks"], stem_t1
        chain = bool(f) and self.fused_chain
        for bi, blk in enumerate(blocks):
            o = pre if pre is not None else E.conv(blk["c1"], x, act_slope=0.0, out_fmt=f)
            pre = None
            nxt = blocks[bi + 1] if bi + 1 < len(blocks) else None
            if (chain and blk["ds"] is None and not blk["feat"] and nxt is not None
                    and E.chain_supported(blk["c2"], blk["c3"], nxt["c1"])):
                sparse = "c3ds" in nxt and nxt["c2"].stride == 2 and not blk["feat"]
                x, pre = E.bottleneck_chain(blk["c2"], blk["c3"], nxt["c1"], o, x, out_even_only=sparse)
                continue
            if "c3ds" in blk and blk["c2"].stride == 1:
                E.conv(blk["c2"], o, cat.slice(0, o.c), act_slope=0.0)
                if chain and nxt is not None and E.chain_supported(None, blk["c3ds"], nxt["c1"], residual=False):
                    x, pre = E.bottleneck_chain(None, blk["c3ds"], nxt["c1"], cat, None)
                else:
                    x = E.conv(blk["c3ds"], cat, act_slope=0.0, out_fmt=f)
                del cat
                continue
            if "c3ds" in blk:
                o = E.conv(blk["c2"], o, act_slope=0.0, out_fmt=f)
                if (chain and not blk["feat"] and nxt is not None
                        and E.chain_supported(None, blk["c3ds"], nxt["c1"], residual=False, cb=x.c)):
                    x, pre = E.bottleneck_chain(None, blk["c3ds"], nxt["c1"], o, None, t1b=x, t1b_stride=blk["c2"].stride)
                    continue
                x = E.conv(blk["c3ds"], o, act_slope=0.0, out_fmt=f, x2=x, x2_stride=blk["c2"].stride)
                if blk["feat"]:
                    feats.append(x)
                continue
            o = E.conv(blk["c2"], o, act_slope=0.0, out_fmt=f)
            if (chain and blk["ds"] is None and nxt is not None and E.chain_supported(None, blk["c3"], nxt["c1"])):
                x, pre = E.bottleneck_chain(None, blk["c3"], nxt["c1"], o, x)
                if blk["feat"]:
                    feats.append(x)
                continue
            idt = x if blk["ds"] is None else E.conv(blk["ds"], x, out_fmt=f)
            x = E.conv(blk["c3"], o, act_slope=0.0, res1=idt, res1_pre=True, out_fmt=f)
            if blk["feat"]:
                feats.append(x)
        if getattr(self, "_debug_feats", None) is not None:
            self._debug_feats.extend(feats)
        o3 = E.conv(p["fpn.output3"], feats[2], act_slope=0.0, out_fmt=f)
        o2 = E.conv(p["fpn.output2"], feats[1], act_slope=0.0, res1=o3, res1_pre=False, out_fmt=f)
        o2 = E.conv(p["fpn.merge2"], o2, act_slope=0.0, out_fmt=f)
        o1 = E.conv(p["fpn.output1"], feats[0], act_slope=0.0, res1=o2, res1_pre=False, out_fmt=f)
        o1 = E.conv(p["fpn.merge1"], o1, act_slope=0.0, out_fmt=f)
        heads = []
        for k, ft in zip((1, 2, 3), (o1, o2, o3)):
            s = E.Act.empty(ft.n, ft.h, ft.w, 384, ft.buf.device, f)
            E.conv(p[f"ssh{k}.ab"], ft, s.slice(0, 192), act_slope=0.0)
            E.conv(p[f"ssh{k}.cd"], s.slice(0, 64), s.slice(256, 128), act_slope=0.0)
            E.conv(p[f"ssh{k}.e"], s.slice(320, 64), s.slice(192, 64), act_slope=0.0)
            heads.append(E.conv(p[f"head{k}"], s.slice(64, 256),
                                None if heads_out is None else heads_out[k - 1]))
        return heads

    def _side_streams(self, dev, k):
        main = E.thread_streams(dev)["main"]
        return E.thread_side_streams(dev, k, with_main=main is not None and torch.cuda.current_stream(dev) == main)

    MAX_OPERAND_BYTES = 0xFFFFFFF0

    def _images_per_launch(self, h: int, w: int) -> int | None:
        if self.precision != 1:
            return None
        hp, wp = ((h - 1) // 2) // 2 + 1, ((w - 1) // 2) // 2 + 1
        return max(1, (self.MAX_OPERAND_BYTES - 1) // (4 * 256 * hp * wp))

    def _streams_for(self, n: int) -> int:
        k = min(self.streams, n // max(1, self.min_images_per_stream))
        return 1 if k < 2 or torch.cuda.is_current_stream_capturing() else k

    def _chunked(self, n: int, h: int, w: int, dev, run, split: bool = True):
        per = self._images_per_launch(h, w)
        q = 1
        while True:
            bounds = [n * i // q for i in range(q + 1)]
            sub = lambda c: -(-c // (self._streams_for(c) if split else 1))
            if per is None or all(sub(b - a) <= per for a, b in zip(bounds[:-1], bounds[1:])):
                break
            q += 1
        if q == 1:
            return run(0, n, None)
        heads = [E.Act.empty(n, -(-h // s), -(-w // s), 32, dev) for s in (8, 16, 32)]
        for a, b in zip(bounds[:-1], bounds[1:]):
            run(a, b, [E.Act(hd.buf[a:b]) for hd in heads])
        return heads

    def _forward_heads_split(self, images_u8: torch.Tensor, heads_out=None):
        n, h, w, _ = images_u8.shape
        k = self._streams_for(n)
        if k < 2:
            return self.forward_heads(None, images_u8, heads_out)
        dev = images_u8.device
        heads = heads_out if heads_out is not None else [E.Act.empty(n, -(-h // s), -(-w // s), 32, dev) for s in (8, 16, 32)]
        cur = torch.cuda.current_stream(dev)
        bounds = [n * i // k for i in range(k + 1)]
        side = self._side_streams(dev, k)
        cus = E.device_props(dev).multi_processor_count // k
        for st, a, b in zip(side, bounds[:-1], bounds[1:]):
            tuned = len(E.Autotune.cache)
            if st != cur:
                st.wait_stream(cur)
            with torch.cuda.stream(st), E.cu_budget(cus):
                self.forward_heads(None, images_u8[a:b], [E.Act(hd.buf[a:b]) for hd in heads])
            if len(E.Autotune.cache) != tuned:
                st.synchronize()
        for st in side:
            if st != cur:
                cur.wait_stream(st)
        return heads

    def detect(self, images_u8: torch.Tensor | None = None, *, x4: E.Act | None = None,
               paddings: torch.Tensor | None = None, max_faces: int | None = None, want_dense: bool = False):
        if self.strategy not in STRATEGIES:
            raise ValueError(f"Unsupported startegy: {self.strategy}")
        fused = x4 is None and "stem_fused" in self._p
        if x4 is None and not fused:
            x4 = E.u8_to_nhwc4(images_u8, sub=(123.0, 117.0, 104.0))
        if fused:
            images_u8 = images_u8.contiguous()
            (n, h, w), dev = images_u8.shape[:3], images_u8.device
            heads = self._chunked(n, h, w, dev, lambda a, b, ho: self._forward_heads_split(images_u8[a:b], ho))
        else:
            n, h, w = x4.n, x4.h, x4.w
            dev = x4.buf.device
            heads = self._chunked(n, h, w, dev, lambda a, b, ho: self.forward_heads(x4 if (a, b) == (0, n) else E.Act(x4.buf[a:b]),
                                                                                    None, ho), split=False)
        P = sum(2 * (-(-h // s)) * (-(-w // s)) for s in (8, 16, 32))
        f32, i32 = torch.float32, torch.int32
        cand_score = torch.empty((n, P), dtype=f32, device=dev)
        cand_box = torch.empty((n, P, 4), dtype=f32, device=dev)
        cand_ldm = torch.empty((n, P, 10), dtype=f32, device=dev)
        cand_prior = torch.empty((n, P), dtype=i32, device=dev)
        cand_count = torch.empty((n,), dtype=i32, device=dev)
        dense = (None, None, None)
        if want_dense:
            dense = (torch.empty((n, P), dtype=f32, device=dev), torch.empty((n, P, 4), dtype=f32, device=dev),
                     torch.empty((n, P, 10), dtype=f32, device=dev))
        if T.ENABLED and not want_dense:
            return self._postprocess_ops(heads, n, h, w, P, paddings, max_faces)
        st = N.stream_ptr()
        lib = N.lib()
        N.check(lib.fcp_retina_decode(heads[0].ptr(), heads[1].ptr(), heads[2].ptr(), n, h, w,
                                      float(self.vis_threshold), float(self.variance[0]), float(self.variance[1]),
                                      N.ptr(cand_score), N.ptr(cand_box), N.ptr(cand_ldm), N.ptr(cand_prior),
                                      N.ptr(cand_count), N.ptr(dense[0]), N.ptr(dense[1]), N.ptr(dense[2]), st),
                "fcp_retina_decode")
        out = nms_select(cand_score, cand_box, cand_count, self.nms_threshold, self.strategy)
        if max_faces is None:
            max_faces = n if self.strategy != "all" else int(out["sel_count"].sum().item())
        max_faces = max(int(max_faces), 1)
        landmarks = torch.empty((max_faces, 5, 2), dtype=f32, device=dev)
        img_idx = torch.empty((max_faces,), dtype=i32, device=dev)
        face_offset = torch.empty((n + 1,), dtype=i32, device=dev)
        if paddings is not None:
            paddings = paddings.to(device=dev, dtype=i32).contiguous()
        N.check(lib.fcp_retina_gather_faces(N.ptr(cand_ldm), N.ptr(out["sel_pos"]), N.ptr(out["sel_count"]), n, P,
                                            N.ptr(paddings), max_faces, N.ptr(face_offset), N.ptr(landmarks),
                                            N.ptr(img_idx), st), "fcp_retina_gather_faces")
        out.update(landmarks=landmarks, img_idx=img_idx, face_offset=face_offset, cand_score=cand_score,
                   cand_box=cand_box, cand_ldm=cand_ldm, cand_prior=cand_prior, cand_count=cand_count,
                   heads=heads, dense=dense, max_faces=max_faces)
        return out

    def _postprocess_ops(self, heads, n, h, w, P, paddings, max_faces):
        ops = T.load()
        dev = heads[0].buf.device
        cand_score, cand_box, cand_ldm, cand_prior, cand_count = ops.retina_decode(
            heads[0].buf, heads[1].buf, heads[2].buf, h, w, float(self.vis_threshold), float(self.variance[0]),
            float(self.variance[1]))
        keep_pos, keep_count, sel_pos, sel_count = ops.nms_select(cand_score, cand_box, cand_count, float(self.nms_threshold),
                                                                  STRATEGIES[self.strategy])
        if max_faces is None:
            max_faces = n if self.strategy != "all" else int(sel_count.sum().item())
        max_faces = max(int(max_faces), 1)
        if paddings is not None:
            paddings = paddings.to(device=dev, dtype=torch.int32).contiguous()
        landmarks, img_idx, face_offset = ops.gather_faces(cand_ldm, sel_pos, sel_count, paddings, max_faces)
        return dict(keep_pos=keep_pos, keep_count=keep_count, sel_pos=sel_pos, sel_count=sel_count, landmarks=landmarks,
                    img_idx=img_idx, face_offset=face_offset, cand_score=cand_score, cand_box=cand_box, cand_ldm=cand_ldm,
                    cand_prior=cand_prior, cand_count=cand_count, heads=heads, dense=(None, None, None), max_faces=max_faces)

    def graphed(self, n: int, h: int, w: int, paddings: torch.Tensor | None = None):
        if self.strategy == "all":
            raise ValueError('graph capture needs a bounded face count: strategy "best" or "largest"')
        key = (n, h, w, None if paddings is None else tuple(paddings.flatten().tolist()))
        cache = self.__dict__.setdefault("_graphs", {})
        if key in cache:
            return cache[key]
        with torch.cuda.device(self.device):
            static = torch.zeros((n, h, w, 3), dtype=torch.uint8, device=self.device)
            prev, E.Autotune.enabled = E.Autotune.enabled, True
            side = torch.cuda.Stream(device=self.device)
            side.wait_stream(torch.cuda.current_stream())
            with torch.cuda.stream(side):
                for _ in range(2):
                    self.detect(static, paddings=paddings, max_faces=n)
            torch.cuda.current_stream().wait_stream(side)
            E.Autotune.enabled = False
            graph = torch.cuda.CUDAGraph()
            with torch.cuda.graph(graph):
                res = self.detect(static, paddings=paddings, max_faces=n)
            E.Autotune.enabled = prev
        cache[key] = (static, res, graph)
        return cache[key]

    @torch.no_grad()
    def predict(self, images: torch.Tensor):
        with torch.cuda.device(self.device):
            if images.dtype == torch.uint8:
                res = self.detect(images.to(self.device).contiguous())
            else:
                x4 = E.f32nchw_to_nhwc4(images.to(self.device, torch.float32), sub=(123.0, 117.0, 104.0))
                res = self.detect(x4=x4)
            nf = int(res["face_offset"][-1].item())
            nf = min(nf, res["max_faces"])
            landmarks = res["landmarks"][:nf].cpu().numpy()
            indices = res["img_idx"][:nf].cpu().numpy().astype(np.int64).tolist()
        return landmarks, indices


def nms_select(cand_score, cand_box, cand_count, nms_threshold=0.4, strategy="all"):
    if strategy not in STRATEGIES:
        raise ValueError(f"Unsupported startegy: {strategy}")
    n, cap = cand_score.shape
    dev = cand_score.device
    i32 = torch.int32
    lib = N.lib()
    ws = torch.empty((int(lib.fcp_retina_nms_workspace_bytes(n, cap)),), dtype=torch.uint8, device=dev)
    keep_pos = torch.empty((n, cap), dtype=i32, device=dev)
    keep_count = torch.empty((n,), dtype=i32, device=dev)
    sel_pos = torch.empty((n, cap), dtype=i32, device=dev)
    sel_count = torch.empty((n,), dtype=i32, device=dev)
    N.check(lib.fcp_retina_nms_select(N.ptr(cand_score), N.ptr(cand_box), N.ptr(cand_count), n, cap,
                                      float(nms_threshold), STRATEGIES[strategy], N.ptr(ws), N.ptr(keep_pos),
                                      N.ptr(keep_count), N.ptr(sel_pos), N.ptr(sel_count), N.stream_ptr()),
            "fcp_retina_nms_select")
    return dict(keep_pos=keep_pos, keep_count=keep_count, sel_pos=sel_pos, sel_count=sel_count)
```

include/fcp_hip.h:

```cpp
#ifndef FCP_HIP_H
#define FCP_HIP_H

#include <stdint.h>

#ifdef __cplusplus
extern "C" {
#endif

#define FCP_ABI_VERSION 15

typedef void* fcp_stream_t;

int fcp_abi_version(void);
const char* fcp_last_error(void);

typedef struct fcp_conv_desc {
  const float* in;
  const void* w;
  const float* bias;
  float* out;
  const float* res1;
  const float* res2;
  const float* wscale;
  const float* in2;
  int32_t n, in_h, in_w;
  int32_t cin, in_ld;
  int32_t in_up2;
  int32_t cout, kh, kw, stride, pad;
  int32_t out_h, out_w, out_ld;
  int32_t tile_n;
  int32_t cin4;
  float act_slope, alpha, alpha2;
  int32_t res1_pre, res1_ld, res1_h, res1_w, res2_ld;
  int32_t precision;
  int32_t in_fmt, out_fmt, res1_fmt, res2_fmt;
  int32_t tile_m;
  int32_t cin2, in2_ld, in2_h, in2_w, in2_stride;
  int32_t flags;
  int32_t cu_budget;
  int32_t band_top, band_bottom;
} fcp_conv_desc;

#define FCP_CONV_FLAT_ADDR 1
#define FCP_CONV_BALANCE_TAIL 2

int fcp_conv2d_nhwc_f32(const fcp_conv_desc* desc, fcp_stream_t stream);

typedef struct fcp_chain_desc {
  const float* t1;
  const void* w2;  const float* ws2;  const float* b2;
  const void* w3;  const float* ws3;  const float* b3;
  const float* res;
  float* out;
  const void* w1n; const float* ws1n; const float* b1n;
  float* t1n;
  const float* t1b;
  int32_t n, h, w, c, cn;
  int32_t t1_ld, res_ld, out_ld, t1n_ld;
  int32_t nout;
  int32_t tile_m;
  int32_t flags;
  int32_t cb, t1b_ld, t1b_h, t1b_w, t1b_stride;
} fcp_chain_desc;
#define FCP_CHAIN_OUT_EVEN_ONLY 1

int fcp_bottleneck_chain_f16x3(const fcp_chain_desc* desc, fcp_stream_t stream);

int fcp_u8_to_nhwc4_f32(const uint8_t* in, float* out, int64_t npix,
                        const float* sub_host, float div, fcp_stream_t stream);

int fcp_f32nchw_to_nhwc4_f32(const float* in, float* out, int n, int h, int w,
                             const float* sub_host, float div, fcp_stream_t stream);

int fcp_maxpool3x3s2_nhwc_f32(const float* in, float* out, int n, int h, int w, int c, int out_ld,
                              int out_h, int out_w, fcp_stream_t stream);
int fcp_maxpool3x3s2_split32(const float* in, float* out, int n, int h, int w, int c, int out_ld,
                             int out_h, int out_w, fcp_stream_t stream);
int fcp_stem7x7s2_relu_pool_u8(const uint8_t* images, int n, int h, int w, const int32_t* mean_rgb,
                               const void* wfrag, const float* bias, const float* wscale, float* out,
                               int out_ld, int out_fmt, fcp_stream_t stream);
int fcp_stem7x7s2_relu_pool_conv1_u8(const uint8_t* images, int n, int h, int w, const int32_t* mean_rgb,
                                     const void* wfrag, const float* bias, const float* wscale, float* out,
                                     int out_ld, int out_fmt, const void* w1, const float* ws1, const float* b1,
                                     float* t1, int t1_ld, fcp_stream_t stream);
int fcp_stem7x7s2_relu_pool_f32(const float* x4, int n, int h, int w, const void* wfrag, const float* bias,
                                const float* wscale, float* out, int out_ld, int out_fmt, fcp_stream_t stream);
int fcp_f32_to_split32(const float* in, float* out, int64_t npix, int c, fcp_stream_t stream);
int fcp_split32_to_f32(const float* in, float* out, int64_t npix, int c, fcp_stream_t stream);
int fcp_absmax_nhwc(const float* x, int64_t npix, int c, int ld, int fmt, float* out_max, fcp_stream_t stream);


int fcp_retina_decode(const float* head0, const float* head1, const float* head2,
                      int n, int img_h, int img_w, float vis_threshold,
                      float var0, float var1,
                      float* cand_score, float* cand_box, float* cand_ldm,
                      int32_t* cand_prior, int32_t* cand_count,
                      float* dense_score, float* dense_box, float* dense_ldm,
                      fcp_stream_t stream);

int64_t fcp_retina_nms_workspace_bytes(int n, int cap);
int fcp_retina_nms_select(const float* cand_score, const float* cand_box,
                          const int32_t* cand_count, int n, int cap,
                          float nms_threshold, int strategy, void* workspace,
                          int32_t* keep_pos, int32_t* keep_count,
                          int32_t* sel_pos, int32_t* sel_count, fcp_stream_t stream);

int fcp_retina_gather_faces(const float* cand_ldm, const int32_t* sel_pos,
                            const int32_t* sel_count, int n, int cap,
                            const int32_t* paddings, int max_faces,
                            int32_t* face_offset, float* out_ldm, int32_t* out_img,
                            fcp_stream_t stream);


int fcp_estimate_transform(const float* src, const float* dst, int f, int k,
                           int allow_skew, double* mat, int32_t* ok, fcp_stream_t stream);

int fcp_estimate_transform_counted(const float* src, const float* dst, int f, int k,
                                   int allow_skew, const int32_t* face_count,
                                   double* mat, int32_t* ok, int64_t* valid_total,
                                   fcp_stream_t stream);

int fcp_warp_affine_u8(const uint8_t* images, int n, int h, int w,
                       const int32_t* img_idx, const double* mat, const int32_t* ok,
                       const int32_t* paddings, int f, int out_h, int out_w, int border,
                       uint8_t* out, fcp_stream_t stream);

int fcp_warp_affine_u8_float(const uint8_t* images, int n, int h, int w,
                             const int32_t* img_idx, const double* mat, const int32_t* ok,
                             const int32_t* paddings, int f, int out_h, int out_w, int border,
                             uint8_t* out, fcp_stream_t stream);

typedef struct fcp_warp_src {
  int64_t off;
  int32_t h, w;
} fcp_warp_src;

int fcp_warp_affine_u8_ragged(const uint8_t* blob, int64_t blob_bytes,
                              const fcp_warp_src* srcs_host, const fcp_warp_src* srcs_dev,
                              const double* mat, const int32_t* ok, int f, int out_h, int out_w,
                              int border, uint8_t* out, fcp_stream_t stream);
int fcp_warp_affine_u8_float_ragged(const uint8_t* blob, int64_t blob_bytes,
                                    const fcp_warp_src* srcs_host, const fcp_warp_src* srcs_dev,
                                    const double* mat, const int32_t* ok, int f, int out_h,
                                    int out_w, int border, uint8_t* out, fcp_stream_t stream);

int fcp_warp_affine_u8_interp(const uint8_t* images, int n, int h, int w,
                              const int32_t* img_idx, const double* mat, const int32_t* ok,
                              const int32_t* paddings, int f, int out_h, int out_w, int border,
                              int interp, uint8_t* out, fcp_stream_t stream);
int fcp_warp_affine_u8_interp_ragged(const uint8_t* blob, int64_t blob_bytes,
                                     const fcp_warp_src* srcs_host, const fcp_warp_src* srcs_dev,
                                     const double* mat, const int32_t* ok, int f, int out_h,
                                     int out_w, int border, int interp, uint8_t* out,
                                     fcp_stream_t stream);

int fcp_warp_interp_weights(int interp, int16_t* out);

int fcp_crop_sharpness_u8(const uint8_t* crops, int f, int h, int w, const int32_t* ok,
                          int64_t* sums, fcp_stream_t stream);

int64_t fcp_jpeg_workspace_bytes(int f, int h, int w, int channels);
int fcp_jpeg_encode_u8(const uint8_t* crops, int f, int h, int w, int channels, int quality, int subsampling,
                       uint8_t* out, int64_t out_stride, int64_t capacity, int32_t* lengths,
                       void* workspace, int64_t workspace_bytes, fcp_stream_t stream);

int64_t fcp_jpeg_workspace_bytes_ex(int f, int h, int w, int channels, int subsampling, int optimize);
int fcp_jpeg_encode_ex_u8(const uint8_t* crops, int f, int h, int w, int channels, int quality,
                          int subsampling, int optimize,
                          uint8_t* out, int64_t out_stride, int64_t capacity, int32_t* lengths,
                          uint8_t* tables, void* workspace, int64_t workspace_bytes, fcp_stream_t stream);

int fcp_jpeg_huffman_tables(const uint32_t* freq, int n, uint8_t* tables, uint32_t* codes, fcp_stream_t stream);

int64_t fcp_png_workspace_bytes(int f, int h, int w, int channels);
int fcp_png_encode_u8(const uint8_t* pixels, int f, int h, int w, int channels,
                      uint8_t* out, int64_t out_stride, int64_t capacity, int32_t* lengths,
                      void* workspace, int64_t workspace_bytes, fcp_stream_t stream);

int fcp_png_huffman_lengths(const uint32_t* freq, int n, uint8_t* lengths, uint32_t* codes, fcp_stream_t stream);

int fcp_matte_u8(const uint8_t* crops, const uint8_t* labels, int f, int h, int w, uint32_t class_bits, int feather,
                 int bg_r, int bg_g, int bg_b, uint8_t* out, uint8_t* alpha, fcp_stream_t stream);

int64_t fcp_matte_blur_workspace_bytes(int f, int h, int w);
int fcp_matte_blur_u8(const uint8_t* crops, const uint8_t* labels, int f, int h, int w, uint32_t class_bits, int feather,
                      const uint16_t* taps, int radius, uint8_t* out, uint8_t* alpha, void* workspace, int64_t workspace_bytes,
                      fcp_stream_t stream);

int64_t fcp_matte_refine_workspace_bytes(int f, int h, int w);
int fcp_matte_refine_u8(const uint8_t* crops, const uint8_t* labels, int f, int h, int w, uint32_t class_bits, int radius, int eps,
                        uint8_t* alpha_out, void* workspace, int64_t workspace_bytes, fcp_stream_t stream);

int fcp_matte_alpha_u8(const uint8_t* crops, const uint8_t* alpha, int f, int h, int w, int bg_r, int bg_g, int bg_b, uint8_t* out,
                       fcp_stream_t stream);
int fcp_matte_blur_alpha_u8(const uint8_t* crops, const uint8_t* labels, const uint8_t* alpha, int f, int h, int w,
                            uint32_t class_bits, const uint16_t* taps, int radius, uint8_t* out, void* workspace,
                            int64_t workspace_bytes, fcp_stream_t stream);

#define FCP_CUTOUT_RGBA 0
#define FCP_CUTOUT_FILL 1
int fcp_feather_alpha_u8(const uint8_t* labels, int f, int h, int w, uint32_t class_bits, int feather, uint8_t* alpha_out,
                         fcp_stream_t stream);
int64_t fcp_cutout_workspace_bytes(int f, int h, int w);
int fcp_cutout_u8(const uint8_t* crops, const uint8_t* alpha, int f, int h, int w, int mode, int bg_r, int bg_g, int bg_b,
                  const uint16_t* taps, int radius, uint8_t* out, void* workspace, int64_t workspace_bytes, fcp_stream_t stream);

int64_t fcp_subject_mask_workspace_bytes(int f, int h, int w);
int fcp_subject_mask_u8(const uint8_t* labels, int f, int h, int w, uint32_t class_bits, int keep_largest, int max_hole, uint8_t* out,
                        void* workspace, int64_t workspace_bytes, fcp_stream_t stream);

int fcp_clahe_u8(const uint8_t* crops, int f, int h, int w, int grid, double clip_limit, uint8_t* luts, uint8_t* out, fcp_stream_t stream);


int fcp_bise_preprocess_u8(const uint8_t* faces, int f, int h, int w, float* out,
                           int out_h, int out_w, const float* mean_host,
                           const float* std_host, fcp_stream_t stream);

int fcp_avgpool_nhwc_f32(const float* in, int n, int hw, int c, int ld, float* out,
                         fcp_stream_t stream);

int fcp_fc_f32(const float* in, const float* w, const float* scale, const float* shift,
               int n, int cin, int cout, int act, float* out, fcp_stream_t stream);

int fcp_scale_add_nhwc_f32(const float* x, int x_ld, const float* scale_nc,
                           const float* add_nc, const float* add_t, int add_t_ld,
                           int n, int hw, int c, float* out, int out_ld, fcp_stream_t stream);

int fcp_parse_tail(const float* logits, int f, int lh, int lw, int ld, int ncls,
                   int mid_h, int mid_w, int out_h, int out_w, uint8_t* labels,
                   int32_t* counts, fcp_stream_t stream);

int fcp_label_mask_u8(const uint8_t* labels, int64_t total, uint32_t class_bits,
                      uint8_t* mask, fcp_stream_t stream);

int fcp_bicubic_down4_u8(const float* x4, int h, int w, int ld, uint8_t* out_rgb,
                         fcp_stream_t stream);

typedef struct fcp_batch_item {
  int64_t src_off;
  int32_t sh, sw;
  int32_t dh, dw;
  int32_t top, left;
  int32_t interp;
  int32_t reserved;
} fcp_batch_item;

int fcp_build_batch_u8(const uint8_t* src_blob, int64_t blob_bytes,
                       const fcp_batch_item* items_host, const fcp_batch_item* items_dev,
                       int n, int out_h, int out_w, int border, uint8_t* out,
                       fcp_stream_t stream);

typedef struct fcp_area_level {
  int64_t src_off;
  int32_t sh, sw;
  int64_t dst_off;
  int32_t dh, dw;
} fcp_area_level;

int fcp_resize_area_ragged_u8(const uint8_t* src_blob, int64_t src_bytes,
                              const fcp_area_level* levels_host, const fcp_area_level* levels_dev,
                              int n, uint8_t* dst_blob, int64_t dst_bytes, fcp_stream_t stream);

#ifdef __cplusplus
}
#endif
#endif
```

Baseline: 1448 faces/s.

## Tile RetinaFace decode across chunks and add small-K LDS NMS path

Replaces the one-block-per-image decode with a two-kernel tiled decode. A count kernel records per-chunk pass bitmasks and counts, and a write kernel computes each chunk's offset and writes the compacted candidates, so many blocks work on each image instead of one. It also adds a small-candidate NMS path that keeps keys, boxes and alive bits in LDS and uses wave-level readlane suppression, and it shares one workspace between decode and NMS. The cost is an extra launch and a workspace round trip for the bitmasks, and postprocess is a small part of the end-to-end pipeline.

```diff
diff --git a/face-crop-plus_amd/_native.py b/face-crop-plus_amd/_native.py
--- a/face-crop-plus_amd/_native.py
+++ b/face-crop-plus_amd/_native.py
@@ -58,6 +58,7 @@
     "fcp_split32_to_f32": [_P, _P, _L, _I, _P],
     "fcp_absmax_nhwc": [_P, _L, _I, _I, _I, _P, _P],
     "fcp_retina_decode": [_P, _P, _P, _I, _I, _I, _F, _F, _F, _P, _P, _P, _P, _P, _P, _P, _P, _P],
+    "fcp_retina_decode_tiled": [_P, _P, _P, _I, _I, _I, _F, _F, _F, _P, _P, _P, _P, _P, _P, _P, _P, _P, _L, _I, _P],
     "fcp_retina_nms_select": [_P, _P, _P, _I, _I, _F, _I, _P, _P, _P, _P, _P, _P],
     "fcp_retina_gather_faces": [_P, _P, _P, _I, _I, _P, _I, _P, _P, _P, _P],
     "fcp_estimate_transform": [_P, _P, _I, _I, _I, _P, _P, _P],
@@ -94,7 +95,8 @@
     "fcp_feather_alpha_u8": [_P, _I, _I, _I, C.c_uint32, _I, _P, _P],
     "fcp_cutout_u8": [_P, _P, _I, _I, _I, _I, _I, _I, _I, _P, _I, _P, _P, _L, _P],
 }
-EXPORTS = ["fcp_abi_version", "fcp_last_error", "fcp_retina_nms_workspace_bytes", "fcp_jpeg_workspace_bytes",
+EXPORTS = ["fcp_abi_version", "fcp_last_error", "fcp_retina_nms_workspace_bytes", "fcp_retina_decode_workspace_bytes",
+           "fcp_jpeg_workspace_bytes",
            "fcp_jpeg_workspace_bytes_ex", "fcp_matte_blur_workspace_bytes", "fcp_matte_refine_workspace_bytes",
            "fcp_subject_mask_workspace_bytes", "fcp_png_workspace_bytes", "fcp_cutout_workspace_bytes"] + list(SIGNATURES)
 
@@ -114,6 +116,8 @@
         raise RuntimeError(f"libfcp_hip.so ABI {l.fcp_abi_version()} != expected {ABI_VERSION}; rebuild")
     l.fcp_retina_nms_workspace_bytes.argtypes = [C.c_int, C.c_int]
     l.fcp_retina_nms_workspace_bytes.restype = C.c_int64
+    l.fcp_retina_decode_workspace_bytes.argtypes = [C.c_int, C.c_int, C.c_int]
+    l.fcp_retina_decode_workspace_bytes.restype = C.c_int64
     l.fcp_jpeg_workspace_bytes.argtypes = [C.c_int, C.c_int, C.c_int, C.c_int]
     l.fcp_jpeg_workspace_bytes.restype = C.c_int64
     l.fcp_jpeg_workspace_bytes_ex.argtypes = [C.c_int] * 6
diff --git a/face-crop-plus_amd/csrc/fcp_retina_post.hip b/face-crop-plus_amd/csrc/fcp_retina_post.hip
--- a/face-crop-plus_amd/csrc/fcp_retina_post.hip
+++ b/face-crop-plus_amd/csrc/fcp_retina_post.hip
@@ -8,6 +8,9 @@
 constexpr int SORT_LDS_KEYS = 8192;
 constexpr int NMS_ALIVE_WORDS = SORT_LDS_KEYS - 256;
 constexpr int NMS_LDS_CAP = NMS_ALIVE_WORDS * 64;
+constexpr int NMS_SMALL_KEYS = 2048;
+static_assert(NMS_SMALL_KEYS + NMS_SMALL_KEYS * 5 / 2 + NMS_SMALL_KEYS / 64 <= NMS_ALIVE_WORDS, "small-K layout: keys | boxes | alive | tile");
+static_assert(NMS_SMALL_KEYS / 2 <= NMS_THREADS, "small-K sort: one pair per thread");
 constexpr int NMS_MAX_CAP = 1 << 26;
 
 struct Levels {
@@ -66,97 +69,184 @@
   }
 }
 
-__global__ void __launch_bounds__(DEC_THREADS) retina_decode_kernel(
-    const float* __restrict__ head0, const float* __restrict__ head1, const float* __restrict__ head2,
-    Levels lv, int img_h, int img_w, float thr, float v0, float v1, float* __restrict__ cand_score,
-    float* __restrict__ cand_box, float* __restrict__ cand_ldm, int* __restrict__ cand_prior,
-    int* __restrict__ cand_count, float* __restrict__ dense_score, float* __restrict__ dense_box,
-    float* __restrict__ dense_ldm) {
-  constexpr int NWAVE = DEC_THREADS / 64;
-  __shared__ int cnt[DEC_MAX_ROUNDS * NWAVE];
+constexpr int DEC_NWAVE = DEC_THREADS / 64;
+constexpr int DEC_CHUNK_DEFAULT = 4096;
+
+struct DecodeArgs {
+  const float *head0, *head1, *head2;
+  Levels lv;
+  int img_h, img_w;
+  float thr, v0, v1;
+  float *cand_score, *cand_box, *cand_ldm;
+  int *cand_prior, *cand_count;
+  float *dense_score, *dense_box, *dense_ldm;
+};
+
+__device__ __forceinline__ unsigned long long decode_pass1(const DecodeArgs& A, int img, int r0, int rounds, int* cnt,
+                                                           unsigned long long* __restrict__ bits) {
+  const int tid = threadIdx.x, lane = tid & 63, wave = tid >> 6;
+  const int P = A.lv.start[3];
+  unsigned long long passbits = 0ull;
+  for (int r = 0; r < rounds; ++r) {
+    const int p = (r0 + r) * DEC_THREADS + tid;
+    bool pass = false;
+    if (p < P) {
+      int l, cell, a;
+      const float* hp = head_cell(A.head0, A.head1, A.head2, A.lv, img, p, l, cell, a);
+      pass = face_score(hp, a) > A.thr;
+    }
+    passbits |= pass ? (1ull << r) : 0ull;
+    const unsigned long long bal = __ballot(pass);
+    if (lane == 0) {
+      cnt[r * DEC_NWAVE + wave] = __popcll(bal);
+      if (bits != nullptr) bits[(r0 + r) * DEC_NWAVE + wave] = bal;
+    }
+  }
+  return passbits;
+}
+
+__device__ __forceinline__ unsigned long long decode_stored_pass1(int r0, int rounds, int* cnt,
+                                                                  const unsigned long long* __restrict__ bits) {
+  const int tid = threadIdx.x, lane = tid & 63, wave = tid >> 6;
+  unsigned long long passbits = 0ull;
+  for (int r = 0; r < rounds; ++r) {
+    const unsigned long long bal = bits[(r0 + r) * DEC_NWAVE + wave];
+    passbits |= ((bal >> lane) & 1ull) << r;
+    if (lane == 0) cnt[r * DEC_NWAVE + wave] = __popcll(bal);
+  }
+  return passbits;
+}
+
+__device__ __forceinline__ int decode_offsets(int* cnt, int n, int carry, int& s_total) {
+  const int tid = threadIdx.x, lane = tid & 63, wave = tid >> 6;
+  __syncthreads();
+  if (wave == 0) {
+    for (int base = 0; base < n; base += 64) {
+      const int idx = base + lane;
+      const int v = idx < n ? cnt[idx] : 0;
+      int incl = v;
+#pragma unroll
+      for (int o = 1; o < 64; o <<= 1) {
+        const int t = __shfl_up(incl, o);
+        if (lane >= o) incl += t;
+      }
+      if (idx < n) cnt[idx] = carry + incl - v;
+      carry += __shfl(incl, 63);
+    }
+    if (lane == 0) s_total = carry;
+  }
+  __syncthreads();
+  return s_total;
+}
+
+__device__ __forceinline__ void decode_pass2(const DecodeArgs& A, int img, int r0, int rounds, const int* cnt,
+                                             unsigned long long passbits) {
+  const int tid = threadIdx.x, lane = tid & 63, wave = tid >> 6;
+  const int P = A.lv.start[3];
+  for (int r = 0; r < rounds; ++r) {
+    const int p = (r0 + r) * DEC_THREADS + tid;
+    const bool pass = (passbits >> r) & 1ull;
+    const unsigned long long bal = __ballot(pass);
+    if (p >= P || (!pass && A.dense_score == nullptr)) continue;
+    int l, cell, a;
+    const float* hp = head_cell(A.head0, A.head1, A.head2, A.lv, img, p, l, cell, a);
+    Decoded dc;
+    decode_prior(hp, A.lv, l, cell, a, A.img_h, A.img_w, A.v0, A.v1, dc);
+    if (A.dense_score != nullptr) {
+      const long d = (long)img * P + p;
+      A.dense_score[d] = dc.score;
+#pragma unroll
+      for (int k = 0; k < 4; ++k) A.dense_box[d * 4 + k] = dc.box[k];
+#pragma unroll
+      for (int k = 0; k < 10; ++k) A.dense_ldm[d * 10 + k] = dc.ldm[k];
+    }
+    if (pass) {
+      const long d = (long)img * P + cnt[r * DEC_NWAVE + wave] + __popcll(bal & ((1ull << lane) - 1ull));
+      A.cand_score[d] = dc.score;
+      A.cand_prior[d] = p;
+#pragma unroll
+      for (int k = 0; k < 4; ++k) A.cand_box[d * 4 + k] = dc.box[k];
+#pragma unroll
+      for (int k = 0; k < 10; ++k) A.cand_ldm[d * 10 + k] = dc.ldm[k];
+    }
+  }
+}
+
+__global__ void __launch_bounds__(DEC_THREADS) retina_decode_kernel(DecodeArgs A) {
+  __shared__ int cnt[DEC_MAX_ROUNDS * DEC_NWAVE];
+  __shared__ int s_total;
   const int img = blockIdx.x;
-  const int tid = threadIdx.x, lane = tid & 63, wave = tid >> 6;
-  const int P = lv.start[3];
-  const int rounds_all = (P + DEC_THREADS - 1) / DEC_THREADS;
-  __shared__ int s_total;
+  const int rounds_all = (A.lv.start[3] + DEC_THREADS - 1) / DEC_THREADS;
   int total = 0;
-
   for (int r0 = 0; r0 < rounds_all; r0 += DEC_MAX_ROUNDS) {
     const int rounds = min(DEC_MAX_ROUNDS, rounds_all - r0);
-    unsigned long long passbits = 0ull;
-    for (int r = 0; r < rounds; ++r) {
-      const int p = (r0 + r) * DEC_THREADS + tid;
-      bool pass = false;
-      if (p < P) {
-        int l, cell, a;
-        const float* hp = head_cell(head0, head1, head2, lv, img, p, l, cell, a);
-        pass = face_score(hp, a) > thr;
-      }
-      passbits |= pass ? (1ull << r) : 0ull;
-      const unsigned long long bal = __ballot(pass);
-      if (lane == 0) cnt[r * NWAVE + wave] = __popcll(bal);
-    }
+    const unsigned long long passbits = decode_pass1(A, img, r0, rounds, cnt, nullptr);
+    total = decode_offsets(cnt, rounds * DEC_NWAVE, total, s_total);
+    decode_pass2(A, img, r0, rounds, cnt, passbits);
     __syncthreads();
-    if (wave == 0) {
-      int carry = total;
-      const int n = rounds * NWAVE;
-      for (int base = 0; base < n; base += 64) {
-        const int idx = base + lane;
-        const int v = idx < n ? cnt[idx] : 0;
-        int incl = v;
-#pragma unroll
-        for (int o = 1; o < 64; o <<= 1) {
-          const int t = __shfl_up(incl, o);
-          if (lane >= o) incl += t;
-        }
-        if (idx < n) cnt[idx] = carry + incl - v;
-        carry += __shfl(incl, 63);
-      }
-      if (lane == 0) s_total = carry;
-    }
-    __syncthreads();
-    total = s_total;
-    for (int r = 0; r < rounds; ++r) {
-      const int p = (r0 + r) * DEC_THREADS + tid;
-      const bool pass = (passbits >> r) & 1ull;
-      const unsigned long long bal = __ballot(pass);
-      if (p >= P || (!pass && dense_score == nullptr)) continue;
-      int l, cell, a;
-      const float* hp = head_cell(head0, head1, head2, lv, img, p, l, cell, a);
-      Decoded dc;
-      decode_prior(hp, lv, l, cell, a, img_h, img_w, v0, v1, dc);
-      if (dense_score != nullptr) {
-        const long d = (long)img * P + p;
-        dense_score[d] = dc.score;
-#pragma unroll
-        for (int k = 0; k < 4; ++k) dense_box[d * 4 + k] = dc.box[k];
-#pragma unroll
-        for (int k = 0; k < 10; ++k) dense_ldm[d * 10 + k] = dc.ldm[k];
-      }
-      if (pass) {
-        const long d = (long)img * P + cnt[r * NWAVE + wave] + __popcll(bal & ((1ull << lane) - 1ull));
-        cand_score[d] = dc.score;
-        cand_prior[d] = p;
-#pragma unroll
-        for (int k = 0; k < 4; ++k) cand_box[d * 4 + k] = dc.box[k];
-#pragma unroll
-        for (int k = 0; k < 10; ++k) cand_ldm[d * 10 + k] = dc.ldm[k];
-      }
-    }
-    __syncthreads();
-  }
-  if (tid == 0) cand_count[img] = total;
+  }
+  if (threadIdx.x == 0) A.cand_count[img] = total;
+}
+
+__global__ void __launch_bounds__(DEC_THREADS) retina_decode_count_kernel(DecodeArgs A, int chunk_rounds, int words,
+                                                                          unsigned long long* __restrict__ ws_bits,
+                                                                          int* __restrict__ ws_count) {
+  __shared__ int cnt[DEC_MAX_ROUNDS * DEC_NWAVE];
+  __shared__ int s_total;
+  const int chunk = blockIdx.x, img = blockIdx.y;
+  const int rounds_all = (A.lv.start[3] + DEC_THREADS - 1) / DEC_THREADS;
+  const int r0 = chunk * chunk_rounds, rounds = min(chunk_rounds, rounds_all - r0);
+  decode_pass1(A, img, r0, rounds, cnt, ws_bits + (long)img * words);
+  const int total = decode_offsets(cnt, rounds * DEC_NWAVE, 0, s_total);
+  if (threadIdx.x == 0) ws_count[img * gridDim.x + chunk] = total;
+}
+
+__global__ void __launch_bounds__(DEC_THREADS) retina_decode_write_kernel(DecodeArgs A, int chunk_rounds, int words,
+                                                                          const unsigned long long* __restrict__ ws_bits,
+                                                                          const int* __restrict__ ws_count) {
+  __shared__ int cnt[DEC_MAX_ROUNDS * DEC_NWAVE];
+  __shared__ int s_total;
+  const int chunk = blockIdx.x, img = blockIdx.y, lane = threadIdx.x & 63;
+  const int rounds_all = (A.lv.start[3] + DEC_THREADS - 1) / DEC_THREADS;
+  const int r0 = chunk * chunk_rounds, rounds = min(chunk_rounds, rounds_all - r0);
+  int base = 0;
+  for (int i = lane; i < chunk; i += 64) base += ws_count[img * gridDim.x + i];
+#pragma unroll
+  for (int o = 32; o > 0; o >>= 1) base += __shfl_xor(base, o);
+  const unsigned long long passbits = decode_stored_pass1(r0, rounds, cnt, ws_bits + (long)img * words);
+  const int total = decode_offsets(cnt, rounds * DEC_NWAVE, base, s_total);
+  decode_pass2(A, img, r0, rounds, cnt, passbits);
+  if (chunk == (int)gridDim.x - 1 && threadIdx.x == 0) A.cand_count[img] = total;
 }
 
 __device__ __forceinline__ void bitonic_pairs(unsigned long long* a, int npairs, int j, int k, int tid,
                                               int nthreads, int index_base) {
   for (int idx = tid; idx < npairs; idx += nthreads) {
-    const int i = 2 * j * (idx / j) + (idx % j);
+    const int i = ((idx & ~(j - 1)) << 1) | (idx & (j - 1));
     const int l = i + j;
     const bool asc = (((i + index_base) & k) == 0);
     const unsigned long long x = a[i], y = a[l];
     if ((x > y) == asc) { a[i] = y; a[l] = x; }
   }
+}
+
+__device__ __forceinline__ void bitonic_sort_small(unsigned long long* a, int Kp, int tid) {
+  for (int k = 2; k <= Kp; k <<= 1)
+    for (int j = k >> 1; j > 0; j >>= 1) {
+      bitonic_pairs(a, Kp >> 1, j, k, tid, NMS_THREADS, 0);
+      const int nj = j > 1 ? j >> 1 : k;
+      if (j > 64 || nj > 64) __syncthreads();
+      else __builtin_amdgcn_fence(__ATOMIC_ACQ_REL, "wavefront");
+    }
+}
+
+__device__ __forceinline__ float lane_value(float v, int src) {
+  return __int_as_float(__builtin_amdgcn_readlane(__float_as_int(v), src));
+}
+__device__ __forceinline__ unsigned long long lane_value(unsigned long long v, int src) {
+  const unsigned lo = (unsigned)__builtin_amdgcn_readlane((int)(unsigned)v, src);
+  const unsigned hi = (unsigned)__builtin_amdgcn_readlane((int)(unsigned)(v >> 32), src);
+  return ((unsigned long long)hi << 32) | lo;
 }
 
 __device__ __forceinline__ bool suppressed(float kx1, float ky1, float kx2, float ky2, float karea,
@@ -168,6 +258,16 @@
   const float a = w * h;
   const float ovr = a / (karea + area - a);
   return !(ovr <= thr);
+}
+
+__device__ __forceinline__ unsigned long long nms_key(float score, int i) {
+  return ((unsigned long long)(~__float_as_uint(score)) << 32) | (unsigned)i;
+}
+
+__device__ __forceinline__ void sorted_box(const float4* box, unsigned long long key, float* out) {
+  const float4 b = box[(int)(unsigned)(key & 0xffffffffull)];
+  const float area = (b.z - b.x + 1.0f) * (b.w - b.y + 1.0f);
+  out[0] = b.x; out[1] = b.y; out[2] = b.z; out[3] = b.w; out[4] = area;
 }
 
 template <bool kGlobalAlive>
@@ -237,6 +337,83 @@
   }
 }
 
+__device__ __forceinline__ void greedy_nms_small(unsigned long long* alive, unsigned long long* sup, float* tile, const float* sbox,
+                                                 const unsigned long long* keys, int* kpos, int K, float thr, int& s_kc,
+                                                 int tid, int lane, int wave) {
+  constexpr int NWAVE = NMS_THREADS / 64;
+  int* tile_n = reinterpret_cast<int*>(tile + 64 * 5);
+  const int ntiles = (K + 63) >> 6;
+  if (tid < ntiles) alive[tid] = (tid << 6) + 64 <= K ? ~0ull : (1ull << (K - (tid << 6))) - 1ull;
+  for (int i = tid; i < (ntiles << 6); i += NMS_THREADS) sup[i] = 0ull;
+  if (tid == 0) s_kc = 0;
+  __syncthreads();
+  {
+    const int split = max(1, NWAVE / ntiles);
+    for (int item = wave; item < ntiles * split; item += NWAVE) {
+      const int t = item / split, part = item - t * split;
+      const int b0 = 64 * part / split, b1 = 64 * (part + 1) / split;
+      const int c = (t << 6) + lane;
+      float x1 = 0.f, y1 = 0.f, x2 = 0.f, y2 = 0.f, area = 0.f;
+      if (c < K) { x1 = sbox[c * 5]; y1 = sbox[c * 5 + 1]; x2 = sbox[c * 5 + 2]; y2 = sbox[c * 5 + 3]; area = sbox[c * 5 + 4]; }
+      unsigned long long m = 0ull;
+      for (int b = b0; b < b1; ++b) {
+        const float kx1 = lane_value(x1, b), ky1 = lane_value(y1, b), kx2 = lane_value(x2, b), ky2 = lane_value(y2, b);
+        const float ka = lane_value(area, b);
+        if (lane > b && suppressed(kx1, ky1, kx2, ky2, ka, x1, y1, x2, y2, area, thr)) m |= 1ull << b;
+      }
+      if (m != 0ull) atomicOr(&sup[c], m);
+    }
+  }
+  __syncthreads();
+
+  for (int t = 0; t < ntiles; ++t) {
+    if (wave == 0) {
+      const int c = (t << 6) + lane;
+      const unsigned long long mine = sup[c];
+      unsigned long long m = 0ull;
+      for (unsigned long long und = lane_value(alive[t], 0); und != 0ull;) {
+        const bool u = (und >> lane) & 1ull;
+        const bool dead = u && (mine & m) != 0ull;
+        const bool keep = u && !dead && (mine & und) == 0ull;
+        const unsigned long long kk = __ballot(keep);
+        m |= kk;
+        und &= ~(kk | __ballot(dead));
+      }
+      const int rank = __popcll(m & ((1ull << lane) - 1ull));
+      const int kc = s_kc;
+      if ((m >> lane) & 1ull) {
+        kpos[kc + rank] = (int)(unsigned)(keys[c] & 0xffffffffull);
+#pragma unroll
+        for (int k = 0; k < 5; ++k) tile[rank * 5 + k] = sbox[c * 5 + k];
+      }
+      if (lane == 0) { *tile_n = __popcll(m); s_kc = kc + __popcll(m); }
+    }
+    __syncthreads();
+    const int nk = *tile_n, nlater = ntiles - (t + 1);
+    if (nk > 0 && nlater > 0) {
+      const int parts = max(1, NWAVE / nlater);
+      for (int item = wave; item < nlater * parts; item += NWAVE) {
+        const int wd = t + 1 + item / parts, part = item - (item / parts) * parts;
+        const int q0 = nk * part / parts, q1 = nk * (part + 1) / parts;
+        const unsigned long long m = __hip_atomic_load(&alive[wd], __ATOMIC_RELAXED, __HIP_MEMORY_SCOPE_WORKGROUP);
+        bool hit = false;
+        if ((m >> lane) & 1ull) {
+          const int c = (wd << 6) + lane;
+          const float x1 = sbox[c * 5], y1 = sbox[c * 5 + 1], x2 = sbox[c * 5 + 2], y2 = sbox[c * 5 + 3];
+          const float area = sbox[c * 5 + 4];
+          for (int q = q0; q < q1 && !hit; ++q) {
+            const float* kb = tile + q * 5;
+            hit = suppressed(kb[0], kb[1], kb[2], kb[3], kb[4], x1, y1, x2, y2, area, thr);
+          }
+        }
+        const unsigned long long hm = __ballot(hit);
+        if (lane == 0 && hm != 0ull) atomicAnd(&alive[wd], ~hm);
+      }
+    }
+    __syncthreads();
+  }
+}
+
 __global__ void __launch_bounds__(NMS_THREADS) retina_nms_kernel(
     const float* __restrict__ cand_score, const float* __restrict__ cand_box,
     const int* __restrict__ cand_count, int cap, int cap_p2, float thr, int strategy,
@@ -244,6 +421,7 @@
     int alive_stride, int* __restrict__ keep_pos,
     int* __restrict__ keep_count, int* __restrict__ sel_pos, int* __restrict__ sel_count) {
   __shared__ unsigned long long lkeys[SORT_LDS_KEYS];
+  __shared__ unsigned long long lsup[NMS_SMALL_KEYS];
   __shared__ int s_kc;
   __shared__ float s_best_area[NMS_THREADS / 64];
   __shared__ int s_best_rank[NMS_THREADS / 64];
@@ -263,12 +441,20 @@
   unsigned long long* gkeys = ws_keys + (long)img * cap_p2;
   float* sbox = ws_box + (long)img * cap_p2 * 5;
 
+  if (Kp <= NMS_SMALL_KEYS) {
+    float* lbox = reinterpret_cast<float*>(lkeys + NMS_SMALL_KEYS);
+    unsigned long long* lalive = lkeys + NMS_SMALL_KEYS + NMS_SMALL_KEYS * 5 / 2;
+    for (int i = tid; i < Kp; i += NMS_THREADS) lkeys[i] = i < K ? nms_key(score[i], i) : ~0ull;
+    __syncthreads();
+    bitonic_sort_small(lkeys, Kp, tid);
+    for (int i = tid; i < K; i += NMS_THREADS) sorted_box(box, lkeys[i], lbox + i * 5);
+    __syncthreads();
+    greedy_nms_small(lalive, lsup, reinterpret_cast<float*>(lkeys + NMS_ALIVE_WORDS), lbox, lkeys, kpos, K, thr, s_kc, tid, lane, wave);
+  } else {
   const bool in_lds = Kp <= SORT_LDS_KEYS;
   unsigned long long* keys = in_lds ? lkeys : gkeys;
   for (int i = tid; i < Kp; i += NMS_THREADS) {
-    unsigned long long kv = ~0ull;
-    if (i < K) kv = ((unsigned long long)(~__float_as_uint(score[i])) << 32) | (unsigned)i;
-    keys[i] = kv;
+    keys[i] = i < K ? nms_key(score[i], i) : ~0ull;
   }
   __syncthreads();
   if (in_lds) {
@@ -299,11 +485,7 @@
   }
   for (int i = tid; i < K; i += NMS_THREADS) {
     const unsigned long long kv = keys[i];
-    const int pos = (int)(unsigned)(kv & 0xffffffffull);
-    const float4 b = box[pos];
-    const float area = (b.z - b.x + 1.0f) * (b.w - b.y + 1.0f);
-    sbox[i * 5 + 0] = b.x; sbox[i * 5 + 1] = b.y; sbox[i * 5 + 2] = b.z; sbox[i * 5 + 3] = b.w;
-    sbox[i * 5 + 4] = area;
+    sorted_box(box, kv, sbox + i * 5);
     if (in_lds) gkeys[i] = kv;
   }
   __threadfence_block();
@@ -313,6 +495,7 @@
     greedy_nms<false>(lkeys, lkeys, sbox, gkeys, kpos, K, thr, s_kc, tid, lane, wave);
   else
     greedy_nms<true>(ws_alive + (long)img * alive_stride, lkeys, sbox, gkeys, kpos, K, thr, s_kc, tid, lane, wave);
+  }
   const int kc = s_kc;
   if (tid == 0) keep_count[img] = kc;
 
@@ -411,27 +594,86 @@
   return (int64_t)n * cap_p2 * (8 + 5 * 4) + (cap > NMS_LDS_CAP ? (int64_t)n * (cap_p2 / 64) * 8 : 0);
 }
 
+namespace {
+
+int decode_args(DecodeArgs& A, const float* head0, const float* head1, const float* head2, int n, int img_h, int img_w,
+                float vis_threshold, float var0, float var1, float* cand_score, float* cand_box, float* cand_ldm,
+                int32_t* cand_prior, int32_t* cand_count, float* dense_score, float* dense_box, float* dense_ldm) {
+  FCP_REQUIRE(head0 && head1 && head2, "retina_decode: null head pointer");
+  FCP_REQUIRE(cand_score && cand_box && cand_ldm && cand_prior && cand_count, "retina_decode: null output");
+  FCP_REQUIRE(n > 0 && img_h > 0 && img_w > 0, "retina_decode: bad sizes");
+  FCP_REQUIRE((dense_score == nullptr) == (dense_box == nullptr) && (dense_box == nullptr) == (dense_ldm == nullptr),
+              "retina_decode: dense outputs must be all set or all NULL");
+  A.head0 = head0; A.head1 = head1; A.head2 = head2;
+  A.lv.start[0] = 0;
+  for (int l = 0; l < 3; ++l) {
+    const int s = 8 << l;
+    A.lv.h[l] = (img_h + s - 1) / s;
+    A.lv.w[l] = (img_w + s - 1) / s;
+    A.lv.start[l + 1] = A.lv.start[l] + 2 * A.lv.h[l] * A.lv.w[l];
+  }
+  A.img_h = img_h; A.img_w = img_w; A.thr = vis_threshold; A.v0 = var0; A.v1 = var1;
+  A.cand_score = cand_score; A.cand_box = cand_box; A.cand_ldm = cand_ldm; A.cand_prior = cand_prior; A.cand_count = cand_count;
+  A.dense_score = dense_score; A.dense_box = dense_box; A.dense_ldm = dense_ldm;
+  return 0;
+}
+
+bool decode_tiling(int P, int chunk_priors, int& chunk_rounds, int& chunks, int& words) {
+  if (chunk_priors == 0) chunk_priors = DEC_CHUNK_DEFAULT;
+  if (chunk_priors < 0 || chunk_priors % DEC_THREADS != 0 || chunk_priors > DEC_MAX_ROUNDS * DEC_THREADS) return false;
+  const int rounds_all = (P + DEC_THREADS - 1) / DEC_THREADS;
+  chunk_rounds = chunk_priors / DEC_THREADS;
+  chunks = (rounds_all + chunk_rounds - 1) / chunk_rounds;
+  words = rounds_all * DEC_NWAVE;
+  return true;
+}
+
+}
+
 extern "C" int fcp_retina_decode(const float* head0, const float* head1, const float* head2, int n,
                                  int img_h, int img_w, float vis_threshold, float var0, float var1,
                                  float* cand_score, float* cand_box, float* cand_ldm, int32_t* cand_prior,
                                  int32_t* cand_count, float* dense_score, float* dense_box,
                                  float* dense_ldm, fcp_stream_t stream) {
-  FCP_REQUIRE(head0 && head1 && head2, "retina_decode: null head pointer");
-  FCP_REQUIRE(cand_score && cand_box && cand_ldm && cand_prior && cand_count, "retina_decode: null output");
-  FCP_REQUIRE(n > 0 && img_h > 0 && img_w > 0, "retina_decode: bad sizes");
-  FCP_REQUIRE((dense_score == nullptr) == (dense_box == nullptr) && (dense_box == nullptr) == (dense_ldm == nullptr),
-              "retina_decode: dense outputs must be all set or all NULL");
-  Levels lv;
-  lv.start[0] = 0;
-  for (int l = 0; l < 3; ++l) {
-    const int s = 8 << l;
-    lv.h[l] = (img_h + s - 1) / s;
-    lv.w[l] = (img_w + s - 1) / s;
-    lv.start[l + 1] = lv.start[l] + 2 * lv.h[l] * lv.w[l];
-  }
-  hipLaunchKernelGGL(retina_decode_kernel, dim3(n), dim3(DEC_THREADS), 0, (hipStream_t)stream, head0, head1,
-                     head2, lv, img_h, img_w, vis_threshold, var0, var1, cand_score, cand_box, cand_ldm,
-                     cand_prior, cand_count, dense_score, dense_box, dense_ldm);
+  DecodeArgs A;
+  if (int rc = decode_args(A, head0, head1, head2, n, img_h, img_w, vis_threshold, var0, var1, cand_score, cand_box,
+                           cand_ldm, cand_prior, cand_count, dense_score, dense_box, dense_ldm)) return rc;
+  hipLaunchKernelGGL(retina_decode_kernel, dim3(n), dim3(DEC_THREADS), 0, (hipStream_t)stream, A);
+  FCP_LAUNCH_OK();
+  return 0;
+}
+
+extern "C" int64_t fcp_retina_decode_workspace_bytes(int n, int priors, int chunk_priors) {
+  int chunk_rounds, chunks, words;
+  if (n <= 0 || priors <= 0 || priors > NMS_MAX_CAP || !decode_tiling(priors, chunk_priors, chunk_rounds, chunks, words)) return 0;
+  return (int64_t)n * words * 8 + (((int64_t)n * chunks * 4 + 7) & ~(int64_t)7);
+}
+
+extern "C" int fcp_retina_decode_tiled(const float* head0, const float* head1, const float* head2, int n,
+                                       int img_h, int img_w, float vis_threshold, float var0, float var1,
+                                       float* cand_score, float* cand_box, float* cand_ldm, int32_t* cand_prior,
+                                       int32_t* cand_count, float* dense_score, float* dense_box, float* dense_ldm,
+                                       void* workspace, int64_t workspace_bytes, int chunk_priors, fcp_stream_t stream) {
+  DecodeArgs A;
+  if (int rc = decode_args(A, head0, head1, head2, n, img_h, img_w, vis_threshold, var0, var1, cand_score, cand_box,
+                           cand_ldm, cand_prior, cand_count, dense_score, dense_box, dense_ldm)) return rc;
+  const int P = A.lv.start[3];
+  int chunk_rounds, chunks, words;
+  FCP_REQUIRE(decode_tiling(P, chunk_priors, chunk_rounds, chunks, words),
+              "retina_decode_tiled: chunk_priors must be 0 or a multiple of %d up to %d, got %d", DEC_THREADS,
+              DEC_MAX_ROUNDS * DEC_THREADS, chunk_priors);
+  FCP_REQUIRE(n <= 65535, "retina_decode_tiled: at most 65535 images per call");
+  FCP_REQUIRE(workspace && ((uintptr_t)workspace & 7) == 0, "retina_decode_tiled: null or misaligned workspace");
+  FCP_REQUIRE(workspace_bytes >= fcp_retina_decode_workspace_bytes(n, P, chunk_priors),
+              "retina_decode_tiled: workspace of %lld bytes, %lld needed", (long long)workspace_bytes,
+              (long long)fcp_retina_decode_workspace_bytes(n, P, chunk_priors));
+  unsigned long long* bits = reinterpret_cast<unsigned long long*>(workspace);
+  int* counts = reinterpret_cast<int*>(bits + (size_t)n * words);
+  hipLaunchKernelGGL(retina_decode_count_kernel, dim3(chunks, n), dim3(DEC_THREADS), 0, (hipStream_t)stream, A,
+                     chunk_rounds, words, bits, counts);
+  FCP_LAUNCH_OK();
+  hipLaunchKernelGGL(retina_decode_write_kernel, dim3(chunks, n), dim3(DEC_THREADS), 0, (hipStream_t)stream, A,
+                     chunk_rounds, words, bits, counts);
   FCP_LAUNCH_OK();
   return 0;
 }
diff --git a/face-crop-plus_amd/csrc/torch_ops/fcp_torch_ops.cpp b/face-crop-plus_amd/csrc/torch_ops/fcp_torch_ops.cpp
--- a/face-crop-plus_amd/csrc/torch_ops/fcp_torch_ops.cpp
+++ b/face-crop-plus_amd/csrc/torch_ops/fcp_torch_ops.cpp
@@ -154,9 +154,18 @@
   return {out, t1n};
 }
 
+static Tensor post_workspace(const c10::optional<Tensor>& given, int64_t bytes, const Tensor& like) {
+  if (!given.has_value()) return at::empty({bytes}, like.options().dtype(at::kByte));
+  const Tensor& ws = *given;
+  TORCH_CHECK(ws.is_cuda() && ws.device() == like.device() && ws.scalar_type() == at::kByte && ws.is_contiguous(),
+              "workspace must be a contiguous uint8 tensor on ", like.device());
+  TORCH_CHECK(ws.numel() >= bytes, "workspace of ", ws.numel(), " bytes, ", bytes, " needed");
+  return ws;
+}
+
 std::tuple<Tensor, Tensor, Tensor, Tensor, Tensor> retina_decode(const Tensor& h0, const Tensor& h1, const Tensor& h2,
                                                                  int64_t img_h, int64_t img_w, double vis, double var0,
-                                                                 double var1) {
+                                                                 double var1, const c10::optional<Tensor>& workspace) {
   dev(h0, "head0", at::kFloat); dev(h1, "head1", at::kFloat); dev(h2, "head2", at::kFloat);
   FCP_DEVICE_GUARD(h0);
   TORCH_CHECK(img_h > 0 && img_w > 0, "image size must be positive");
@@ -177,15 +186,16 @@
   auto i = h0.options().dtype(at::kInt);
   Tensor score = at::empty({n, P}, f), box = at::empty({n, P, 4}, f), ldm = at::empty({n, P, 10}, f);
   Tensor prior = at::empty({n, P}, i), count = at::empty({n}, i);
-  ok(fcp_retina_decode(h0.data_ptr<float>(), h1.data_ptr<float>(), h2.data_ptr<float>(), (int)n, (int)img_h, (int)img_w,
-                       (float)vis, (float)var0, (float)var1, score.data_ptr<float>(), box.data_ptr<float>(),
-                       ldm.data_ptr<float>(), prior.data_ptr<int>(), count.data_ptr<int>(), nullptr, nullptr, nullptr,
-                       cur_stream()), "fcp::retina_decode");
+  Tensor ws = post_workspace(workspace, fcp_retina_decode_workspace_bytes((int)n, (int)P, 0), h0);
+  ok(fcp_retina_decode_tiled(h0.data_ptr<float>(), h1.data_ptr<float>(), h2.data_ptr<float>(), (int)n, (int)img_h, (int)img_w,
+                             (float)vis, (float)var0, (float)var1, score.data_ptr<float>(), box.data_ptr<float>(),
+                             ldm.data_ptr<float>(), prior.data_ptr<int>(), count.data_ptr<int>(), nullptr, nullptr, nullptr,
+                             ws.data_ptr(), ws.numel(), 0, cur_stream()), "fcp::retina_decode");
   return {score, box, ldm, prior, count};
 }
 
 std::tuple<Tensor, Tensor, Tensor, Tensor> nms_select(const Tensor& score, const Tensor& box, const Tensor& count,
-                                                      double thr, int64_t strategy) {
+                                                      double thr, int64_t strategy, const c10::optional<Tensor>& workspace) {
   dev(score, "cand_score", at::kFloat); dev(box, "cand_box", at::kFloat); dev(count, "cand_count", at::kInt);
   FCP_DEVICE_GUARD(score);
   TORCH_CHECK(score.dim() == 2, "cand_score is (n, cap)");
@@ -195,7 +205,7 @@
   TORCH_CHECK(count.dim() == 1 && count.size(0) == n, "cand_count must be (", n, ",), got ", count.sizes());
   TORCH_CHECK(strategy >= 0 && strategy <= 2, "strategy: 0 all, 1 best, 2 largest");
   auto i = score.options().dtype(at::kInt);
-  Tensor ws = at::empty({fcp_retina_nms_workspace_bytes((int)n, (int)cap)}, score.options().dtype(at::kByte));
+  Tensor ws = post_workspace(workspace, fcp_retina_nms_workspace_bytes((int)n, (int)cap), score);
   Tensor keep_pos = at::empty({n, cap}, i), keep_count = at::empty({n}, i), sel_pos = at::empty({n, cap}, i), sel_count = at::empty({n}, i);
   ok(fcp_retina_nms_select(score.data_ptr<float>(), box.data_ptr<float>(), count.data_ptr<int>(), (int)n, (int)cap, (float)thr,
                            (int)strategy, ws.data_ptr(), keep_pos.data_ptr<int>(), keep_count.data_ptr<int>(),
@@ -683,9 +693,10 @@
   m.def("bottleneck_chain(Tensor t1, int t1_c0, Tensor? res, int res_c0, Tensor? w2, Tensor? ws2, Tensor? b2, Tensor w3, Tensor ws3, "
         "Tensor b3, Tensor? w1n, Tensor? ws1n, Tensor? b1n, int c, int nout, int cn, int tile_m=0, int flags=0, Tensor? t1b=None, "
         "int t1b_c0=0, int cb=0, int t1b_stride=1) -> (Tensor, Tensor)");
-  m.def("retina_decode(Tensor head0, Tensor head1, Tensor head2, int img_h, int img_w, float vis, float var0, float var1) "
+  m.def("retina_decode(Tensor head0, Tensor head1, Tensor head2, int img_h, int img_w, float vis, float var0, float var1, "
+        "Tensor(a!)? workspace=None) "
         "-> (Tensor, Tensor, Tensor, Tensor, Tensor)");
-  m.def("nms_select(Tensor cand_score, Tensor cand_box, Tensor cand_count, float nms_threshold, int strategy) "
+  m.def("nms_select(Tensor cand_score, Tensor cand_box, Tensor cand_count, float nms_threshold, int strategy, Tensor(a!)? workspace=None) "
         "-> (Tensor, Tensor, Tensor, Tensor)");
   m.def("gather_faces(Tensor cand_ldm, Tensor sel_pos, Tensor sel_count, Tensor? paddings, int max_faces) -> (Tensor, Tensor, Tensor)");
   m.def("similarity_from_5pt(Tensor src, Tensor dst, bool allow_skew, Tensor? face_count=None, Tensor(a!)? valid_total=None) "
diff --git a/face-crop-plus_amd/retinaface.py b/face-crop-plus_amd/retinaface.py
--- a/face-crop-plus_amd/retinaface.py
+++ b/face-crop-plus_amd/retinaface.py
@@ -295,12 +295,14 @@
             return self._postprocess_ops(heads, n, h, w, P, paddings, max_faces)
         st = N.stream_ptr()
         lib = N.lib()
-        N.check(lib.fcp_retina_decode(heads[0].ptr(), heads[1].ptr(), heads[2].ptr(), n, h, w,
-                                      float(self.vis_threshold), float(self.variance[0]), float(self.variance[1]),
-                                      N.ptr(cand_score), N.ptr(cand_box), N.ptr(cand_ldm), N.ptr(cand_prior),
-                                      N.ptr(cand_count), N.ptr(dense[0]), N.ptr(dense[1]), N.ptr(dense[2]), st),
-                "fcp_retina_decode")
-        out = nms_select(cand_score, cand_box, cand_count, self.nms_threshold, self.strategy)
+        ws = post_workspace(n, P, dev)
+        N.check(lib.fcp_retina_decode_tiled(heads[0].ptr(), heads[1].ptr(), heads[2].ptr(), n, h, w,
+                                            float(self.vis_threshold), float(self.variance[0]), float(self.variance[1]),
+                                            N.ptr(cand_score), N.ptr(cand_box), N.ptr(cand_ldm), N.ptr(cand_prior),
+                                            N.ptr(cand_count), N.ptr(dense[0]), N.ptr(dense[1]), N.ptr(dense[2]),
+                                            N.ptr(ws), ws.numel(), 0, st),
+                "fcp_retina_decode_tiled")
+        out = nms_select(cand_score, cand_box, cand_count, self.nms_threshold, self.strategy, workspace=ws)
         if max_faces is None:
             max_faces = n if self.strategy != "all" else int(out["sel_count"].sum().item())
         max_faces = max(int(max_faces), 1)
@@ -320,11 +322,12 @@
     def _postprocess_ops(self, heads, n, h, w, P, paddings, max_faces):
         ops = T.load()
         dev = heads[0].buf.device
+        ws = post_workspace(n, P, dev)
         cand_score, cand_box, cand_ldm, cand_prior, cand_count = ops.retina_decode(
             heads[0].buf, heads[1].buf, heads[2].buf, h, w, float(self.vis_threshold), float(self.variance[0]),
-            float(self.variance[1]))
+            float(self.variance[1]), ws)
         keep_pos, keep_count, sel_pos, sel_count = ops.nms_select(cand_score, cand_box, cand_count, float(self.nms_threshold),
-                                                                  STRATEGIES[self.strategy])
+                                                                  STRATEGIES[self.strategy], ws)
         if max_faces is None:
             max_faces = n if self.strategy != "all" else int(sel_count.sum().item())
         max_faces = max(int(max_faces), 1)
@@ -374,14 +377,24 @@
         return landmarks, indices
 
 
-def nms_select(cand_score, cand_box, cand_count, nms_threshold=0.4, strategy="all"):
+def post_workspace(n, cap, dev):
+    lib = N.lib()
+    size = max(int(lib.fcp_retina_nms_workspace_bytes(n, cap)), int(lib.fcp_retina_decode_workspace_bytes(n, cap, 0)))
+    return torch.empty((size,), dtype=torch.uint8, device=dev)
+
+
+def nms_select(cand_score, cand_box, cand_count, nms_threshold=0.4, strategy="all", workspace=None):
     if strategy not in STRATEGIES:
         raise ValueError(f"Unsupported startegy: {strategy}")
     n, cap = cand_score.shape
     dev = cand_score.device
     i32 = torch.int32
     lib = N.lib()
-    ws = torch.empty((int(lib.fcp_retina_nms_workspace_bytes(n, cap)),), dtype=torch.uint8, device=dev)
+    ws = workspace
+    if ws is None:
+        ws = torch.empty((int(lib.fcp_retina_nms_workspace_bytes(n, cap)),), dtype=torch.uint8, device=dev)
+    elif ws.numel() < int(lib.fcp_retina_nms_workspace_bytes(n, cap)) or ws.dtype != torch.uint8 or ws.device != dev:
+        raise ValueError("nms_select: workspace too small, not uint8 or on another device")
     keep_pos = torch.empty((n, cap), dtype=i32, device=dev)
     keep_count = torch.empty((n,), dtype=i32, device=dev)
     sel_pos = torch.empty((n, cap), dtype=i32, device=dev)
diff --git a/include/fcp_hip.h b/include/fcp_hip.h
--- a/include/fcp_hip.h
+++ b/include/fcp_hip.h
@@ -98,6 +98,16 @@
                       float* dense_score, float* dense_box, float* dense_ldm,
                       fcp_stream_t stream);
 
+int64_t fcp_retina_decode_workspace_bytes(int n, int priors, int chunk_priors);
+int fcp_retina_decode_tiled(const float* head0, const float* head1, const float* head2,
+                            int n, int img_h, int img_w, float vis_threshold,
+                            float var0, float var1,
+                            float* cand_score, float* cand_box, float* cand_ldm,
+                            int32_t* cand_prior, int32_t* cand_count,
+                            float* dense_score, float* dense_box, float* dense_ldm,
+                            void* workspace, int64_t workspace_bytes, int chunk_priors,
+                            fcp_stream_t stream);
+
 int64_t fcp_retina_nms_workspace_bytes(int n, int cap);
 int fcp_retina_nms_select(const float* cand_score, const float* cand_box,
                           const int32_t* cand_count, int n, int cap,
```

Result: no change. 1454 faces/s (median of 6 runs) (+0.4%).
